# ml-unito/PartitionedLS.jl

Hardware: AMD Instinct MI355X
Metric: sign-pattern NNLS solves/sec (whole node); fp64 obj gap vs ref (higher is better)
Workload: dtype f64

## Files before the change

partitionedls.jl_amd/csrc/api.hip:

```cpp
#include "ctx.h"
#include <cstdarg>
#include <cstdio>
#include <cstdlib>
#include <cstring>
#include <new>

namespace partls {

static thread_local char g_err[512] = "";
static thread_local bool g_runtime_gone = false;
bool runtime_gone() { return g_runtime_gone; }
void set_error(const char *fmt, ...)
{
    va_list ap;
    va_start(ap, fmt);
    vsnprintf(g_err, sizeof(g_err), fmt, ap);
    va_end(ap);
}

void t_begin(partls_ctx *c, int w) { (void)hipEventRecord(c->ev0[w], c->stream); }
void t_end(partls_ctx *c, int w) { (void)hipEventRecord(c->ev1[w], c->stream); c->timed[w] = true; }
void t_collect(partls_ctx *c)
{
    for (int w = 0; w < PARTLS_T_COUNT; ++w)
        if (c->timed[w]) {
            float f = 0.f;
            if (hipEventElapsedTime(&f, c->ev0[w], c->ev1[w]) == hipSuccess) c->ms[w] = (double)f;
            c->timed[w] = false;
        }
}

partls_status check_common(partls_ctx *c, const void *X, int64_t N, int64_t M, int64_t ldX, const void *P, int64_t K, int64_t ldP)
{
    if (!c) { set_error("context is NULL"); return PARTLS_ERR_BAD_ARG; }
    if (!X || !P) { set_error("X or P is NULL"); return PARTLS_ERR_BAD_ARG; }
    if (N < 1 || M < 1 || K < 1) { set_error("need N, M, K >= 1 (got %lld, %lld, %lld)", (long long)N, (long long)M, (long long)K); return PARTLS_ERR_BAD_ARG; }
    if (ldX < N || ldP < M) { set_error("leading dimension smaller than the row count"); return PARTLS_ERR_BAD_ARG; }
    if (ldX >= ((int64_t)1 << 30)) { set_error("ldX = %lld: this build supports leading dimensions below 2^30 rows", (long long)ldX); return PARTLS_ERR_UNSUPPORTED; }
    if (K > 61) { set_error("K = %lld groups: this build supports K <= 61 (Alt, BnB, predict) and K <= 39 for the enumeration of fit(Opt)", (long long)K); return PARTLS_ERR_UNSUPPORTED; }
    if (M + 1 > 1023) { set_error("M = %lld features: this build supports M <= 1022", (long long)M); return PARTLS_ERR_UNSUPPORTED; }
    return PARTLS_OK;
}

double h_reg(const partls_ctx *c, int a, int b)
{
    double v = c->hG[(size_t)a * c->ldg + b];
    if (c->eta != 0.0 && a <= c->M && b <= c->M) v += c->eta * (double)__builtin_popcountll(c->mask_aug[a] & c->mask_aug[b]);
    return v;
}

}

using namespace partls;

extern "C" {

int partls_version(void) { return 105; }
const char *partls_last_error(void) { return g_err; }

int partls_device_count(void)
{
    int n = 0;
    if (hipGetDeviceCount(&n) != hipSuccess) return 0;
    return n;
}

partls_status partls_create(int device, partls_ctx **out)
try {
    if (!out) { set_error("partls_create: out is NULL"); return PARTLS_ERR_BAD_ARG; }
    *out = nullptr;
    int n = partls_device_count();
    if (n <= 0 || device < 0 || device >= n) {
        set_error("partls_create: no usable HIP device (count=%d, requested=%d); this library has no CPU fallback", n, device);
        return PARTLS_ERR_NO_DEVICE;
    }
    PARTLS_HIP_CHECK(hipSetDevice(device));
    partls_ctx *c = new (std::nothrow) partls_ctx();
    if (!c) { set_error("out of host memory"); return PARTLS_ERR_BAD_ARG; }
    c->device = device;
    if (hipDeviceGetAttribute(&c->ncu, hipDeviceAttributeMultiprocessorCount, device) != hipSuccess || c->ncu < 1) c->ncu = 256;
    if (const char *e = getenv("PARTLS_TOL_REL")) c->knobs.tol_rel = atof(e);
    if (const char *e = getenv("PARTLS_CHAIN_LEN")) c->knobs.chain_len = atoll(e);
    if (const char *e = getenv("PARTLS_GRID")) c->knobs.grid = atoll(e);
    if (const char *e = getenv("PARTLS_GRAM_S")) c->knobs.gram_S = atoi(e);
    if (const char *e = getenv("PARTLS_GRAM_CR")) c->knobs.gram_cr = atoi(e);
    if (const char *e = getenv("PARTLS_COOP_ROWS")) c->knobs.coop_rows = atoi(e);
    if (const char *e = getenv("PARTLS_PAIR")) c->knobs.pair = atoi(e) != 0 ? 1 : 0;
    if (const char *e = getenv("PARTLS_BIT_ORDER")) c->knobs.bit_order = !strcmp(e, "identity") ? 1 : (!strcmp(e, "calibrate") ? 2 : 0);
    if (const char *e = getenv("PARTLS_ALT_MS_MAX_ROUNDS")) c->knobs.alt_ms_max_rounds = atoi(e);
    if (const char *e = getenv("PARTLS_ALT_MS_CHUNK")) c->knobs.alt_ms_chunk = atoll(e);
    if (const char *e = getenv("PARTLS_KKT_TOL")) c->knobs.kkt_tol = atof(e);
    if (const char *e = getenv("PARTLS_NEAR_TIE_REL")) c->knobs.near_tie_rel = atof(e);
    if (const char *e = getenv("PARTLS_CAL_WB")) c->knobs.cal_wb = atof(e);
    if (const char *e = getenv("PARTLS_CAL_WS")) c->knobs.cal_ws = atof(e);
    c->knobs.no_coop = getenv("PARTLS_NO_COOP") != nullptr;
    c->knobs.no_export = getenv("PARTLS_NO_EXPORT") != nullptr;
    c->knobs.no_staged_upload = getenv("PARTLS_NO_STAGED_UPLOAD") != nullptr;
    if (const char *e = getenv("PARTLS_REG_MAXT")) { const int v = atoi(e); if (v >= 1 && v <= 20) c->knobs.reg_maxt = v; }
    c->knobs.eager_generic = getenv("PARTLS_EAGER_GENERIC") != nullptr;
    c->knobs.bnb_cold = getenv("PARTLS_BNB_COLD") != nullptr;
    if (const char *e = getenv("PARTLS_BNB_BATCH")) c->knobs.bnb_batch = atoi(e);
    if (const char *e = getenv("PARTLS_BNB_POOL_MB")) c->knobs.bnb_pool_mb = atoi(e);
    if (const char *e = getenv("PARTLS_BNB_WG_PER_CU")) c->knobs.bnb_wg_per_cu = atoi(e);
    if (const char *e = getenv("PARTLS_COOP_FAULT")) c->knobs.coop_fault = atoi(e);
    c->knobs.lz_fault = getenv("PARTLS_LZ_FAULT") != nullptr;
    c->knobs.no_tab_refine = getenv("PARTLS_NO_TAB_REFINE") != nullptr;
    c->knobs.finish_trace = getenv("PARTLS_FINISH_TRACE") != nullptr;
    c->knobs.alt_trace = getenv("PARTLS_ALT_TRACE") != nullptr;
    c->knobs.alt_always_check = getenv("PARTLS_ALT_ALWAYS_CHECK") != nullptr;
    c->knobs.print_stamps = getenv("PARTLS_PRINT_STAMPS") != nullptr;
    c->knobs.cv_serial = getenv("PARTLS_CV_SERIAL") != nullptr && strcmp(getenv("PARTLS_CV_SERIAL"), "0") != 0;
    c->knobs.resample_serial = getenv("PARTLS_RESAMPLE_SERIAL") != nullptr && strcmp(getenv("PARTLS_RESAMPLE_SERIAL"), "0") != 0;
    hipError_t e = hipStreamCreateWithFlags(&c->stream, hipStreamNonBlocking);
    for (int w = 0; w < PARTLS_T_COUNT && e == hipSuccess; ++w) {
        e = hipEventCreate(&c->ev0[w]);
        if (e == hipSuccess) e = hipEventCreate(&c->ev1[w]);
    }
    if (e != hipSuccess) {
        set_error("partls_create: stream / event creation failed: %s", hipGetErrorString(e));
        partls_destroy(c);
        return PARTLS_ERR_HIP;
    }
    *out = c;
    return PARTLS_OK;
}
PARTLS_ABI_GUARD

void partls_destroy(partls_ctx *c)
{
    if (!c) return;
    partls_destroy(c->cv_work);
    for (partls_ctx *v : c->cv_view) partls_destroy(v);
    c->cv_work = nullptr;
    c->cv_view.clear();
    int ndev = 0;
    const bool alive = hipGetDeviceCount(&ndev) == hipSuccess && ndev > c->device && hipSetDevice(c->device) == hipSuccess;
    if (alive && c->stream) (void)hipStreamSynchronize(c->stream);
    const hipStream_t stream = c->stream;
    hipEvent_t ev[2 * PARTLS_T_COUNT];
    for (int w = 0; w < PARTLS_T_COUNT; ++w) { ev[2 * w] = c->ev0[w]; ev[2 * w + 1] = c->ev1[w]; }
    g_runtime_gone = !alive;
    delete c;
    g_runtime_gone = false;
    if (alive) {
        for (hipEvent_t e : ev) if (e) (void)hipEventDestroy(e);
        if (stream) (void)hipStreamDestroy(stream);
    }
}

static partls_status predict_common(partls_ctx *c, const void *X, int64_t N, int64_t M, int64_t ldX, int x_on_device,
                                    const int64_t *P, int64_t K, int64_t ldP, const double *alpha, const double *beta, double t,
                                    double *yhat, bool x_f32 = false)
{
    partls_status st = check_common(c, X, N, M, ldX, P, K, ldP);
    if (st != PARTLS_OK) return st;
    if (!alpha || !beta || !yhat) { set_error("partls_predict: NULL argument"); return PARTLS_ERR_BAD_ARG; }
    PARTLS_HIP_CHECK(hipSetDevice(c->device));
    std::vector<double> w((size_t)M, 0.0);
    for (int64_t m = 0; m < M; ++m) {
        double s = 0.0;
        for (int64_t k = 0; k < K; ++k) {
            const int64_t v = P[m + k * ldP];
            if (v != 0 && v != 1) { set_error("P has an entry outside {0,1}"); return PARTLS_ERR_BAD_PARTITION; }
            s += (double)v * alpha[m] * beta[k];
        }
        w[(size_t)m] = s;
    }
    PARTLS_HIP_CHECK(c->wdev.ensure((size_t)(M + 1) * sizeof(double)));
    PARTLS_HIP_CHECK(hipMemcpyAsync(c->wdev.p, w.data(), (size_t)M * sizeof(double), hipMemcpyHostToDevice, c->stream));
    const void *dX = X;
    int64_t ld = ldX;
    double *dyh = yhat;
    if (!x_on_device) {
        const size_t esz = x_f32 ? sizeof(float) : sizeof(double);
        PARTLS_HIP_CHECK(c->predX.ensure((size_t)N * M * esz));
        PARTLS_HIP_CHECK(c->predY.ensure((size_t)N * sizeof(double)));
        const partls_status us = upload_matrix(c, c->predX.p, X, N, M, ldX, esz);
        if (us != PARTLS_OK) return us;
        dX = c->predX.p; ld = N; dyh = c->predY.as<double>();
    }
    PARTLS_HIP_CHECK(launch_residual(dX, N, M, ld, nullptr, c->wdev.as<double>(), t, nullptr, 1024, dyh, c->stream, nullptr, x_f32));
    if (!x_on_device)
        PARTLS_HIP_CHECK(hipMemcpyAsync(yhat, c->predY.p, (size_t)N * sizeof(double), hipMemcpyDeviceToHost, c->stream));
    PARTLS_HIP_CHECK(hipStreamSynchronize(c->stream));
    if (!x_on_device) { c->predX.release(); c->predY.release(); }
    return PARTLS_OK;
}

partls_status partls_predict(partls_ctx *c, const double *X, int64_t N, int64_t M, int64_t ldX, const int64_t *P, int64_t K,
                             int64_t ldP, const double *alpha, const double *beta, double t, double *yhat)
try {
    return predict_common(c, X, N, M, ldX, 0, P, K, ldP, alpha, beta, t, yhat);
}
PARTLS_ABI_GUARD

partls_status partls_predict_device(partls_ctx *c, const double *dX, int64_t N, int64_t M, int64_t ldX, const int64_t *P,
                                    int64_t K, int64_t ldP, const double *alpha, const double *beta, double t, double *dyhat)
try {
    return predict_common(c, dX, N, M, ldX, 1, P, K, ldP, alpha, beta, t, dyhat);
}
PARTLS_ABI_GUARD

partls_status partls_predict_f32(partls_ctx *c, const float *X, int64_t N, int64_t M, int64_t ldX, const int64_t *P, int64_t K,
                                 int64_t ldP, const double *alpha, const double *beta, double t, double *yhat)
try {
    return predict_common(c, X, N, M, ldX, 0, P, K, ldP, alpha, beta, t, yhat, true);
}
PARTLS_ABI_GUARD

partls_status partls_predict_device_f32(partls_ctx *c, const float *dX, int64_t N, int64_t M, int64_t ldX, const int64_t *P,
                                        int64_t K, int64_t ldP, const double *alpha, const double *beta, double t, double *dyhat)
try {
    return predict_common(c, dX, N, M, ldX, 1, P, K, ldP, alpha, beta, t, dyhat, true);
}
PARTLS_ABI_GUARD

partls_status partls_synth_truth(uint64_t seed, int64_t D, int64_t K, int64_t *P, double *wstar)
try {
    if (D < 1 || K < 1 || K > D) { set_error("partls_synth_truth: bad D/K"); return PARTLS_ERR_BAD_ARG; }
    std::vector<int64_t> grp((size_t)D);
    int64_t j = 0;
    for (int64_t k = 0; k < K; ++k) {
        const int64_t sz = D / K + ((k < D % K) ? 1 : 0);
        for (int64_t q = 0; q < sz; ++q) grp[(size_t)j++] = k;
    }
    if (P) {
        memset(P, 0, (size_t)D * K * sizeof(int64_t));
        for (int64_t m = 0; m < D; ++m) P[m + grp[(size_t)m] * D] = 1;
    }
    auto uni = [&](uint64_t stream, uint64_t idx) { return (double)(rnd64(seed, stream, idx) >> 11) * 0x1.0p-53; };
    if (wstar)
        for (int64_t k = 0; k < K; ++k) {
            double sum = 0.0;
            for (int64_t m = 0; m < D; ++m) if (grp[(size_t)m] == k) sum += uni(2, (uint64_t)m);
            const double bk = (uni(3, (uint64_t)k) - 0.5) * 10.0;
            for (int64_t m = 0; m < D; ++m) if (grp[(size_t)m] == k) wstar[m] = (uni(2, (uint64_t)m) / sum) * bk;
        }
    return PARTLS_OK;
}
PARTLS_ABI_GUARD

partls_status partls_synth_device(partls_ctx *c, uint64_t seed, int64_t N, int64_t D, const double *wstar, double *dX, double *dy)
try {
    if (!c || !wstar || !dX || !dy || N < 1 || D < 1) { set_error("partls_synth_device: bad argument"); return PARTLS_ERR_BAD_ARG; }
    PARTLS_HIP_CHECK(hipSetDevice(c->device));
    PARTLS_HIP_CHECK(c->wdev.ensure((size_t)D * sizeof(double)));
    PARTLS_HIP_CHECK(hipMemcpyAsync(c->wdev.p, wstar, (size_t)D * sizeof(double), hipMemcpyHostToDevice, c->stream));
    PARTLS_HIP_CHECK(launch_synth(seed, N, D, c->wdev.as<double>(), dX, dy, c->stream));
    PARTLS_HIP_CHECK(hipStreamSynchronize(c->stream));
    return PARTLS_OK;
}
PARTLS_ABI_GUARD

partls_status partls_get_timing(const partls_ctx *c, partls_timer which, double *ms)
try {
    if (!c || !ms || (int)which < 0 || (int)which >= PARTLS_T_COUNT) { set_error("partls_get_timing: bad argument"); return PARTLS_ERR_BAD_ARG; }
    *ms = c->ms[(int)which];
    return PARTLS_OK;
}
PARTLS_ABI_GUARD

partls_status partls_get_upload(const partls_ctx *c, double *ms, double *bytes)
try {
    if (!c || !ms || !bytes) { set_error("partls_get_upload: bad argument"); return PARTLS_ERR_BAD_ARG; }
    *ms = c->last_upload_ms; *bytes = c->last_upload_bytes;
    return PARTLS_OK;
}
PARTLS_ABI_GUARD

partls_status partls_get_pivots(const partls_ctx *c, int64_t *pivots)
try {
    if (!c || !pivots) { set_error("partls_get_pivots: bad argument"); return PARTLS_ERR_BAD_ARG; }
    *pivots = (int64_t)c->last_pivots;
    return PARTLS_OK;
}
PARTLS_ABI_GUARD

partls_status partls_get_kkt_violation(const partls_ctx *c, double *violation, double *min_pivot)
try {
    if (!c || !violation) { set_error("partls_get_kkt_violation: bad argument"); return PARTLS_ERR_BAD_ARG; }
    *violation = c->last_kkt;
    if (min_pivot) *min_pivot = c->last_min_loo;
    return PARTLS_OK;
}
PARTLS_ABI_GUARD

partls_status partls_get_vetoes(const partls_ctx *c, int64_t *vetoes)
try {
    if (!c || !vetoes) { set_error("partls_get_vetoes: bad argument"); return PARTLS_ERR_BAD_ARG; }
    *vetoes = (int64_t)c->last_vetoes;
    return PARTLS_OK;
}
PARTLS_ABI_GUARD

partls_status partls_get_blocks(const partls_ctx *c, int64_t *blocks)
try {
    if (!c || !blocks) { set_error("partls_get_blocks: bad argument"); return PARTLS_ERR_BAD_ARG; }
    *blocks = (int64_t)c->last_blocks;
    return PARTLS_OK;
}
PARTLS_ABI_GUARD

partls_status partls_get_sweep_route(const partls_ctx *c, int *kernel, int *tiles)
try {
    if (!c || !kernel || !tiles) { set_error("partls_get_sweep_route: bad argument"); return PARTLS_ERR_BAD_ARG; }
    const partls_ctx *p = c->prepared ? c : (c->cv_work && c->cv_work->prepared ? c->cv_work : nullptr);
    if (!p) { set_error("partls_get_sweep_route: context not prepared"); return PARTLS_ERR_STATE; }
    *kernel = p->use_reg ? (sweep_reg_small(p->T) ? PARTLS_ROUTE_REG_256 : PARTLS_ROUTE_REG_512)
                         : (p->knobs.eager_generic ? PARTLS_ROUTE_EAGER : PARTLS_ROUTE_DEFERRED);
    *tiles = p->use_reg ? p->T : 0;
    return PARTLS_OK;
}
PARTLS_ABI_GUARD

partls_status partls_get_near_ties(const partls_ctx *c, int64_t *evaluated)
try {
    if (!c || !evaluated) { set_error("partls_get_near_ties: bad argument"); return PARTLS_ERR_BAD_ARG; }
    *evaluated = c->last_near_evaluated;
    return PARTLS_OK;
}
PARTLS_ABI_GUARD

partls_status partls_get_gram(const partls_ctx *c, double *G_aug)
try {
    if (!c || !c->prepared || !G_aug) { set_error("partls_get_gram: context not prepared"); return PARTLS_ERR_STATE; }
    const int na = (int)c->M + 2;
    for (int j = 0; j < na; ++j)
        for (int i = 0; i < na; ++i) G_aug[(size_t)i + (size_t)j * na] = h_reg(c, i, j);
    return PARTLS_OK;
}
PARTLS_ABI_GUARD

}
```

partitionedls.jl_amd/csrc/common.h:

```cpp
#pragma once
#include <hip/hip_runtime.h>
#include <stdint.h>
#include <new>
#include <vector>
#include <string>
#include "../../include/partls.h"

namespace partls {

void set_error(const char *fmt, ...);
#define PARTLS_HIP_CHECK(expr)                                                                      \
    do {                                                                                            \
        hipError_t _e = (expr);                                                                     \
        if (_e != hipSuccess) {                                                                     \
            ::partls::set_error("%s failed: %s (%s:%d)", #expr, hipGetErrorString(_e), __FILE__, __LINE__); \
            return PARTLS_ERR_HIP;                                                                  \
        }                                                                                           \
    } while (0)
#define PARTLS_ABI_GUARD                                                                                                          \
    catch (const std::bad_alloc &) { ::partls::set_error("out of host memory"); return PARTLS_ERR_BAD_ARG; }                      \
    catch (...) { ::partls::set_error("internal error: an exception reached the C ABI"); return PARTLS_ERR_BAD_ARG; }

struct BitOrder { uint8_t gbit[40]; };

struct SweepParams {
    int n;
    int kbits;
    const uint64_t *mask;
    const double *T0;
    double *scratch;
    int64_t g_begin, g_end;
    int64_t chain_len;
    double tol;
    double piv_eps;
    int max_rounds;
    int pair;
    double *all_opt;
    double *best_obj;
    int64_t *best_pat;
    double *best_sol;
    double *second_obj;
    int64_t *second_pat;
    BitOrder rbit;
    unsigned long long *n_unconverged;
    unsigned long long *n_pivots;
    unsigned long long *n_vetoes;
    const int8_t *node_code;
    double *node_sol;
    double *node_obj2;
    int node_ld;
    double *node_tab;
    int8_t *node_basic;
    unsigned *node_piv;
    const double *const *node_src;
    double *const *node_dst;
    int resume;
    unsigned *grid_ctr;
    int coop_fault;
    int64_t batch_t0, batch_out;
    const double *batch_tol;
};

__device__ __forceinline__ bool ref_index_less(unsigned long long a, unsigned long long b, const unsigned char *rbit)
{
    unsigned long long d = a ^ b;
    int top = -1, at = 0;
    while (d) {
        const int i = __builtin_ctzll(d);
        d &= d - 1;
        const int r = rbit[i];
        if (r > top) { top = r; at = i; }
    }
    return top >= 0 && !((a >> at) & 1ULL);
}

hipError_t launch_sweep_generic(const SweepParams &p, int grid, hipStream_t s, bool models = false);
hipError_t launch_sweep_lazy(const SweepParams &p, int grid, hipStream_t s, bool models = false);
hipError_t launch_sweep_blk(const SweepParams &p, int T, int grid, hipStream_t s, bool models = false);
hipError_t launch_sweep_blk_batch(const SweepParams &p, int T, int grid, int batch, hipStream_t s);
hipError_t launch_layout_reg_batch(const double *Tfull, int n, int T, int batch, double *T0reg, hipStream_t s);
hipError_t launch_sweep_coop(const SweepParams &p, int nwg, hipStream_t s);
bool       sweep_reg_supported(int n);
int        sweep_reg_tiles(int n);
bool       sweep_reg_exports(int T);
bool       sweep_reg_small(int T);
size_t     sweep_reg_t0_doubles(int T);
int        sweep_reg_concurrency(int T);
hipError_t launch_layout_reg(const double *Tfull, int n, int T, double *T0reg, hipStream_t s);

size_t     gram_slab_doubles(int64_t N, int64_t M, int gram_S, int gram_cr, int *chunks_out, int *ldg_out);
hipError_t launch_gram(const void *X, int64_t N, int64_t M, int64_t ldX, const double *y, double *slab, int chunks,
                       int ldg, int gram_S, int gram_cr, double *G, hipStream_t s, const double *sw = nullptr, bool x_f32 = false);
hipError_t launch_gram_weightings(const double *X, int64_t N, int64_t M, int64_t ldX, const double *y, double *slab, int64_t slab_stride,
                                  int chunks, int ldg, int gram_S, int gram_cr, double *G, int64_t gstride, const double *sw, int batch,
                                  hipStream_t s);
int        weight_prep_blocks(int64_t N);
hipError_t launch_weightings_prep(const double *W, int64_t N, int64_t ldW, int batch, double *S, double *part, hipStream_t st);
inline hipError_t launch_weight_prep(const double *w, int64_t N, double *s, double *part, hipStream_t st) { return launch_weightings_prep(w, N, N, 1, s, part, st); }
hipError_t launch_oob_sse(const double *X, int64_t N, int64_t M, int64_t ldX, const double *y, const double *W, int64_t ldW,
                          const double *wv, int batch, double *part, hipStream_t st);

hipError_t launch_prep(const double *G, int ldg, int M, double eta, const uint64_t *mask_aug, int free_intercept,
                       const int *perm, double *scale, double *Tfull, int n, hipStream_t s);
hipError_t launch_prep_batch(const double *G, int64_t gstride, int E, int64_t q0, const double *eta, int ldg, int M, const uint64_t *mask_aug,
                             int free_intercept, const int *perm, double tol_rel, double *scale, double *Tfull, double *tol, int n,
                             int batch, hipStream_t s);

int        walk_flipped_bit(int chain, int step, int kbits, int seg_len, int nseg);
hipError_t launch_walk_codes(const uint64_t *mask, int n, int kbits, int chains, int L, int seg_len, int nseg, int8_t *codes, hipStream_t s);
hipError_t launch_pattern_gather(const double *in, int64_t npat, int kbits, const BitOrder &order, double *out, hipStream_t s);

hipError_t launch_models_cleanup(double *sol, const double *obj, int64_t g0, int64_t cnt, int M, int K, int kbits, const BitOrder &order,
                                 bool order_identity, const int *perm, const double *scale, const uint64_t *mask_aug, bool want_raw,
                                 double *out, hipStream_t s);

hipError_t launch_bnb_codes(const uint64_t *mask_tab, int n, const uint64_t *pat, const uint64_t *free_, int cnt, int8_t *codes, hipStream_t s);
hipError_t launch_bnb_nu(const double *sol, const double *obj2, int n, const double *scale, const uint64_t *mask_tab, int Kp,
                         const uint64_t *free_, int cnt, double *lb, int *branch, hipStream_t s);

hipError_t launch_gersh(const double *Tfull, int n, double *out, hipStream_t s);
hipError_t launch_alt_beta_system(const double *G, int ldg, int M, double eta, const uint64_t *mask_aug, const double *a, int Kp,
                                  double *GA, double *Hg, hipStream_t s);
hipError_t launch_alt_beta_system_batch(const double *G, int ldg, int M, double eta, const uint64_t *mask_aug, const double *a, int Kp,
                                        const int *slot, int cnt, double *GA, double *Hg, hipStream_t s);
hipError_t launch_alt_beta_system_problems(const double *G, int64_t gstride, int E, int64_t q0, const double *eta, const int *prob, int ldg,
                                           int M, const uint64_t *mask_aug, const double *a, int Kp, const int *slot, int cnt, double *GA,
                                           double *Hg, hipStream_t s);
hipError_t launch_residual(const void *X, int64_t N, int64_t M, int64_t ldX, const double *y, const double *w, double t,
                           double *partial, int nblocks, double *yhat, hipStream_t s, const double *wt = nullptr, bool x_f32 = false);
int        xtr_slices(int64_t N);
hipError_t launch_xtr(const void *X, int64_t N, int64_t M, int64_t ldX, const double *y, const double *yhat, double *gpart,
                      hipStream_t s, const double *wt = nullptr, bool x_f32 = false);
hipError_t launch_synth(uint64_t seed, int64_t N, int64_t D, const double *wstar_dev, double *X, double *y, hipStream_t s);

uint64_t rnd64(uint64_t seed, uint64_t stream, uint64_t idx);

}
```

partitionedls.jl_amd/csrc/ctx.h:

```cpp
#pragma once
#include "common.h"
#include <functional>
#include <vector>

namespace partls {

bool runtime_gone();
struct NoCopy {
    NoCopy() = default;
    NoCopy(const NoCopy &) = delete;
    NoCopy &operator=(const NoCopy &) = delete;
};

struct DevBuf : NoCopy {
    void *p = nullptr;
    size_t bytes = 0;
    ~DevBuf() { release(); }
    hipError_t ensure(size_t b)
    {
        if (b <= bytes && p) return hipSuccess;
        if (p) { hipError_t e = hipFree(p); p = nullptr; bytes = 0; if (e != hipSuccess) return e; }
        hipError_t e = hipMalloc(&p, b ? b : 8);
        if (e == hipSuccess) bytes = b;
        return e;
    }
    void release() { if (p && !runtime_gone()) (void)hipFree(p); p = nullptr; bytes = 0; }
    template <class T> T *as() const { return static_cast<T *>(p); }
};

struct DevChunks : NoCopy {
    std::vector<void *> v;
    ~DevChunks() { release(); }
    void release() { if (!runtime_gone()) for (void *q : v) (void)hipFree(q); v.clear(); }
    size_t size() const { return v.size(); }
    void push_back(void *q) { v.push_back(q); }
    void *operator[](size_t i) const { return v[i]; }
};

struct PinnedDoubles : NoCopy {
    double *p = nullptr;
    size_t cap = 0, n = 0, cap_prev = 0;
    ~PinnedDoubles() { release(); }
    hipError_t resize(size_t count)
    {
        if (count > cap) {
            if (p) (void)hipHostFree(p);
            p = nullptr; cap = 0;
            size_t want = count > 512 ? count : 512;
            if (want < 2 * cap_prev) want = 2 * cap_prev;
            hipError_t e = hipHostMalloc((void **)&p, want * sizeof(double), hipHostMallocDefault);
            if (e != hipSuccess) return e;
            cap = cap_prev = want;
        }
        n = count;
        return hipSuccess;
    }
    void release() { if (p && !runtime_gone()) (void)hipHostFree(p); p = nullptr; cap = n = 0; }
    double *data() const { return p; }
    size_t size() const { return n; }
    double &operator[](size_t i) const { return p[i]; }
};

template <class T> struct PinnedArray : NoCopy {
    T *p = nullptr;
    ~PinnedArray() { release(); }
    hipError_t alloc(size_t count)
    {
        release();
        const hipError_t e = hipHostMalloc((void **)&p, count * sizeof(T), hipHostMallocDefault);
        if (e != hipSuccess) p = nullptr;
        return e;
    }
    void release() { if (p && !runtime_gone()) (void)hipHostFree(p); p = nullptr; }
    operator T *() const { return p; }
};

struct UploadStaging : NoCopy {
    char *pin[8] = {};
    hipStream_t stream[4] = {};
    hipEvent_t event[8] = {};
    ~UploadStaging()
    {
        if (runtime_gone()) return;
        for (int i = 0; i < 8; ++i) { if (pin[i]) (void)hipHostFree(pin[i]); if (event[i]) (void)hipEventDestroy(event[i]); }
        for (int t = 0; t < 4; ++t) if (stream[t]) (void)hipStreamDestroy(stream[t]);
    }
};

}

struct partls_knobs {
    double tol_rel = 1e-11;
    long long chain_len = 0;
    long long grid = 0;
    int gram_S = 0, gram_cr = 0;
    int coop_rows = 0;
    bool no_coop = false;
    int reg_maxt = 18;
    bool no_staged_upload = false;
    bool no_export = false;
    bool eager_generic = false;
    int bnb_batch = 1024;
    int bnb_pool_mb = 65536;
    int bnb_wg_per_cu = 8;
    bool bnb_cold = false;
    bool lz_fault = false;
    int coop_fault = 0;
    bool no_tab_refine = false;
    bool finish_trace = false;
    bool alt_trace = false;
    bool alt_always_check = false;
    bool print_stamps = false;
    int alt_ms_max_rounds = 0;
    long long alt_ms_chunk = 0;
    double kkt_tol = 1e-12;
    double near_tie_rel = 1e-13;
    double cal_wb = 1.0, cal_ws = 1.0;
    bool cv_serial = false;
    bool resample_serial = false;
    int pair = -1;
    int bit_order = 0;
};

struct partls_ctx {
    int device = 0;
    int ncu = 256;
    partls_knobs knobs;
    hipStream_t stream = nullptr;
    hipEvent_t ev0[PARTLS_T_COUNT] = {}, ev1[PARTLS_T_COUNT] = {};
    bool timed[PARTLS_T_COUNT] = {};
    double ms[PARTLS_T_COUNT] = {};

    bool prepared = false;
    int64_t N = 0, M = 0, K = 0, ldX = 0;
    double eta = 0.0;
    uint32_t flags = 0;
    bool faithful = false;
    const void *dX = nullptr;
    bool x_f32 = false;
    const double *dy = nullptr;
    partls::DevBuf ownX, ownY;
    const double *dw = nullptr, *ds = nullptr;
    partls::DevBuf ownW, ownS, wPart;
    bool multi_rank = false;
    std::vector<int64_t> P;
    std::vector<uint64_t> mask_aug;
    std::vector<uint64_t> pack;
    const uint64_t *maskTabP = nullptr;
    const int *permP = nullptr;
    int ldg = 0, chunks = 0;
    partls::DevBuf slab, G, maskAugD , scale, Tfull, T0reg, scratch, bestObj, bestSol , bestPat, counters, allOpt,
        wdev, partial, yhatD, gD, nodeCode, nodeSol, nodeObj, predX, predY, gridCtr, nodeTab, nodeBasic, altA, altGA, altHg,
        nodePiv, maskInt, allOptRef, bnbIn, bnbOut, altGersh, amsState, amsWork;
    partls::DevChunks bnbChunks;
    size_t bnbSlotBytes = 0, bnbMaxSlots = 0;
    int bnbChunkSlots = 512;
    std::vector<int> bnbFree, bnbRefs;
    std::vector<partls_ctx *> peers;
    partls::PinnedDoubles hPart, hGpart;
    partls::PinnedDoubles sweepOut, nodeOut, exportSol;
    partls::DevBuf mdlRows, mdlOut, mdlCtr;
    partls::PinnedDoubles mdlStage;
    std::function<partls_status(partls_ctx *)> gram_hook;
    partls::PinnedDoubles amsHostIn, amsHostOut;
    partls::PinnedDoubles bnbHostIn, bnbHostOut;
    partls::UploadStaging up;
    double last_upload_ms = 0.0, last_upload_bytes = 0.0;
    partls::PinnedDoubles hG;
    partls::PinnedDoubles hScale;
    int n = 0, kbits = 0, T = 0;
    std::vector<int> perm;
    std::vector<uint64_t> mask_tab;
    bool use_reg = false;
    partls::BitOrder order{};
    bool order_ready = false, order_identity = true;
    std::vector<double> flip_cost;
    double tol = 0.0;
    unsigned long long last_pivots = 0, last_vetoes = 0, last_blocks = 0;
    std::vector<int64_t> near_pat;
    int64_t near_for = -1;
    std::vector<std::pair<double, int64_t>> cand;
    int64_t last_near_evaluated = 0;
    int export_wg = -1;
    double last_kkt = 0.0;
    double last_min_loo = 0.0;
    unsigned long long sweep_vetoes = 0;
    bool coop_state_valid = false;
    bool coop_fallback = false;
    partls::PinnedArray<double> hTab;
    partls::PinnedArray<int8_t> hBasic;
    size_t hTabDoubles = 0;
    bool tab_valid = false, tab_full = false;
    partls_ctx *cv_work = nullptr;
    std::vector<partls_ctx *> cv_view;
    partls::DevBuf cvG, cvBatch, cvEta;
    partls::PinnedDoubles cvHost, cvHostG;
    partls::DevBuf rsW, rsS, rsPart, rsWv;
    partls::PinnedDoubles rsHost;
};

namespace partls {

void t_begin(partls_ctx *c, int w);
void t_end(partls_ctx *c, int w);
void t_collect(partls_ctx *c);

partls_status ctx_prepare(partls_ctx *c, const void *X, int64_t N, int64_t M, int64_t ldX, const double *y, int x_on_device,
                          const int64_t *P, int64_t K, int64_t ldP, double eta, bool faithful, uint32_t flags, const double *w = nullptr,
                          bool x_f32 = false);
void forget_problem(partls_ctx *c);
partls_status adopt_or_upload(partls_ctx *c, const void *X, int64_t N, int64_t M, int64_t ldX, const double *y, int x_on_device, size_t esz);
partls_status prepare_weights(partls_ctx *c, const double *w, int64_t N, int on_device);
partls_status ctx_prepare_tableau(partls_ctx *c);
partls_status load_partition(partls_ctx *c, const int64_t *P, int64_t M, int64_t K, int64_t ldP);
partls_status upload_matrix(partls_ctx *c, void *dst, const void *X, int64_t N, int64_t M, int64_t ldX, size_t esz = sizeof(double));
constexpr double SWEEP_PIV_EPS = 1e-11;
inline int sweep_max_rounds(int n) { return 20 * (n + 1); }
SweepParams sweep_params(const partls_ctx *c, bool internal_order);
partls_status ensure_sweep_scratch(partls_ctx *c, int grid);
partls_status node_sweep_params(partls_ctx *c, size_t nodes, int64_t chain_len, int grid, SweepParams *p);
inline void bind_counters(SweepParams &p, unsigned long long *w) { p.n_unconverged = w; p.n_pivots = w + 1; p.n_vetoes = w + 2; }
struct SweepBlock { unsigned long long *counters; double *best_obj; int64_t *best_pat; double *second_obj; int64_t *second_pat; };
inline size_t sweep_block_words(int grid, bool runner_up) { return 4 + (runner_up ? 4 : 2) * (size_t)grid; }
inline SweepBlock sweep_block(double *base, int grid, bool runner_up)
{
    double *b = base + 4;
    const size_t g = (size_t)grid;
    return {reinterpret_cast<unsigned long long *>(base), b, reinterpret_cast<int64_t *>(b + g), runner_up ? b + 2 * g : nullptr,
            runner_up ? reinterpret_cast<int64_t *>(b + 3 * g) : nullptr};
}
void bind_sweep_block(SweepParams &p, double *base, int grid, bool runner_up);
hipError_t launch_any_sweep(partls_ctx *c, SweepParams &p, int grid, bool models = false);
partls_status calibrate_bit_order(partls_ctx *c);
bool sweep_plan(partls_ctx *c, int64_t total, int64_t *chain_len_out, int *grid_out, const char *who);
bool sweep_pairs(const partls_ctx *c, int64_t total);
int64_t reference_pattern(const partls_ctx *c, int64_t q);
void install_sweep_result(partls_ctx *c, const double *sweep_out, int grid, bool has_sol, double *bobj_out, int64_t *bpat_out);

struct CvOut {
    std::vector<double> alpha, beta, t, opt, sse;
    std::vector<int64_t> best;
    std::vector<int32_t> status;
    void assign(int64_t B, int64_t M, int64_t K);
    void deliver(int64_t B, int64_t M, int64_t K, double *alpha_out, int64_t ld_alpha, double *beta_out, int64_t ld_beta, double *t_out,
                 double *opt_out, int64_t *best_out, double *sse_out, int32_t *status_out) const;
};
struct ProblemBatch {
    int64_t B = 0, E = 1;
    const double *eta = nullptr;
    const double *G = nullptr, *hostG = nullptr;
    int64_t gs = 0;
    bool serial = false;
    const char *who = "";
    std::function<partls_status(int64_t q, int64_t bpat, int64_t unconv)> finish;
};
partls_status make_internal(partls_ctx *c, partls_ctx **slot);
partls_status cv_check_inputs(const char *who, partls_ctx *c, const double *X, int64_t N, int64_t M, int64_t ldX, const double *y,
                              const int64_t *P, int64_t K, int64_t ldP, const int64_t *fold_ptr, int64_t F, const double *eta, int64_t E);
partls_status cv_grams(partls_ctx *c, const double *X, int64_t N, int64_t M, int64_t ldX, const double *y, const double *w, int x_on_device,
                       int64_t K, const int64_t *fold_ptr, int64_t F, uint32_t flags, const char *who, int *ldg_out, int *chunks_out);
void cv_point_rows(partls_ctx *c, partls_ctx *W, const int64_t *fold_ptr, int64_t F, int64_t f);
void batch_reset(partls_ctx *c, int64_t N, int64_t M, int64_t K, uint32_t flags);
partls_status batch_calibrate(partls_ctx *c, const int64_t *P, int64_t ldP, uint32_t flags, int ldg, int chunks, const ProblemBatch &pb,
                              int64_t cal_gram, const std::function<void(partls_ctx *)> &point_rows);
partls_status batch_sweep(partls_ctx *c, const ProblemBatch &pb);
partls_status finish_model(partls_ctx *c, int64_t q, int64_t bpat, int64_t unconv, CvOut &o);
void model_weights(const partls_ctx *work, const CvOut &o, int64_t q, double *w);

partls_status solve_nodes(partls_ctx *c, const std::vector<int8_t> &codes, size_t cnt, std::vector<double> &sols,
                          std::vector<double> &obj2, unsigned long long *unconv, bool resume = false, bool want_tab = false);
partls_status solve_nodes_device(partls_ctx *c, size_t cnt, const int8_t *code, double *obj2, double *sol,
                                 unsigned long long *counters, int max_rounds);
partls_status solve_nodes_device_at(partls_ctx *c, const double *T0reg, double tol, size_t cnt, const int8_t *code, double *obj2,
                                    double *sol, unsigned long long *counters, int max_rounds);

struct AltProblems {
    int64_t B = 1, E = 1, q0 = 0;
    const double *G = nullptr;
    int64_t gs = 0;
    const double *eta = nullptr;
    const double *scale = nullptr;
    const double *T0reg = nullptr;
    size_t t0d = 0;
    const double *tol = nullptr;
    const double *yy = nullptr;
};
struct AltTables {
    double *alpha_all; int64_t ld_alpha_all; double *beta_all; int64_t ld_beta_all;
    double *t_all, *opt_all; int64_t *iters_all; int32_t *status_all;
};
struct AltWinner {
    int64_t start = -1, iters = 0;
    double opt = 0.0;
    std::vector<double> a, b, wv, hdiag;
    std::vector<int8_t> vcode;
};
partls_status alt_multistart_core(partls_ctx *c, const AltProblems *pp, double eps, int64_t T, int64_t R,
                                  const double *alpha0, int64_t ld_alpha0, const double *beta0, int64_t ld_beta0,
                                  const AltTables &tb, AltWinner *win);
partls_status alt_finish(partls_ctx *c, const std::vector<double> &a, const std::vector<double> &b, const std::vector<double> &wv,
                         const std::vector<int8_t> &vcode_last, const std::vector<double> &hdiag, const std::vector<double> &gersh,
                         double optval, int64_t iters_done, unsigned long long unconv_total,
                         double *alpha, double *beta, double *t, double *opt, int64_t *iters);
void opt_codes(const partls_ctx *c, uint64_t pattern, std::vector<int8_t> &codes);

void unscale_solution(const partls_ctx *c, const double *sol, std::vector<double> &w);
partls_status data_pass(partls_ctx *c, const std::vector<double> &w, bool want_obj, bool want_grad, double *obj2, std::vector<double> *g,
                        const std::function<void()> &overlap);
partls_status data_objective(partls_ctx *c, const std::vector<double> &w, double *opt, std::vector<double> *grad = nullptr);
bool kkt_says_ill_conditioned(const partls_ctx *c);
double kkt_violation_data(const partls_ctx *c, const std::vector<double> &w, const std::vector<double> &g, const std::vector<int8_t> &code,
                          int *worst);
struct RefineOut { bool have = false; double obj = 0.0; std::vector<double> g; };
partls_status refine_solution(partls_ctx *c, std::vector<double> &w, bool free_intercept, int steps = 2, RefineOut *out = nullptr);
double h_reg(const partls_ctx *c, int a, int b);
partls_status check_common(partls_ctx *c, const void *X, int64_t N, int64_t M, int64_t ldX, const void *P, int64_t K, int64_t ldP);

}
```

partitionedls.jl_amd/csrc/opt.hip:

```cpp
#include "ctx.h"
#include "near_tie.h"
#include "sweep_rules.h"
#include <algorithm>
#include <chrono>
#include <cmath>
#include <cstdio>
#include <cstring>
#include <functional>
#include <thread>

namespace partls {

static bool opt_range_ok(const partls_ctx *c, const char *who)
{
    if (c->kbits <= 40) return true;
    set_error("%s: %d sign bits: the enumeration of 2^(K+1) patterns is out of range (K <= 39); fit(Alt) and fit(BnB) take up to 61 groups", who, c->kbits);
    return false;
}

static void cleanup_opt(const partls_ctx *c, const std::vector<double> &w, uint64_t pattern, double *alpha, double *beta, double *t)
{
    const int64_t M = c->M, K = c->K;
    std::vector<double> a((size_t)M, 0.0);
    for (int64_t m = 0; m < M; ++m) {
        const int f = sign_of_var(c->mask_aug[(size_t)m], pattern);
        a[(size_t)m] = (f != 0) ? w[(size_t)m] / (double)f : 0.0;
        if (a[(size_t)m] < 0.0) a[(size_t)m] = 0.0;
    }
    std::vector<double> A((size_t)K, 0.0);
    for (int64_t k = 0; k < K; ++k) {
        double s = 0.0;
        for (int64_t m = 0; m < M; ++m) s += (double)c->P[(size_t)m + (size_t)k * M] * a[(size_t)m];
        const double sk = ((pattern >> k) & 1ULL) ? 1.0 : -1.0;
        beta[k] = sk * s;
        A[(size_t)k] = (s == 0.0) ? 1.0 : s;
    }
    for (int64_t m = 0; m < M; ++m) {
        double s = 0.0;
        for (int64_t k = 0; k < K; ++k) s += (double)c->P[(size_t)m + (size_t)k * M] * a[(size_t)m] / A[(size_t)k];
        alpha[m] = s;
    }
    *t = w[(size_t)M];
}

}

using namespace partls;

extern "C" {

partls_status partls_opt_prepare(partls_ctx *c, const double *X, int64_t N, int64_t M, int64_t ldX, const double *y,
                                 int x_on_device, const int64_t *P, int64_t K, int64_t ldP, double eta, uint32_t flags)
try {
    return ctx_prepare(c, X, N, M, ldX, y, x_on_device, P, K, ldP, eta, (flags & PARTLS_OPT_FAITHFUL_INTERCEPT) != 0, flags);
}
PARTLS_ABI_GUARD

partls_status partls_opt_prepare_weighted(partls_ctx *c, const double *X, int64_t N, int64_t M, int64_t ldX, const double *y,
                                          const double *w, int x_on_device, const int64_t *P, int64_t K, int64_t ldP, double eta,
                                          uint32_t flags)
try {
    return ctx_prepare(c, X, N, M, ldX, y, x_on_device, P, K, ldP, eta, (flags & PARTLS_OPT_FAITHFUL_INTERCEPT) != 0, flags, w);
}
PARTLS_ABI_GUARD

partls_status partls_opt_prepare_f32(partls_ctx *c, const float *X, int64_t N, int64_t M, int64_t ldX, const double *y, const double *w,
                                     int x_on_device, const int64_t *P, int64_t K, int64_t ldP, double eta, uint32_t flags)
try {
    return ctx_prepare(c, X, N, M, ldX, y, x_on_device, P, K, ldP, eta, (flags & PARTLS_OPT_FAITHFUL_INTERCEPT) != 0, flags, w, true);
}
PARTLS_ABI_GUARD

int64_t partls_opt_num_patterns(const partls_ctx *c) { return (c && c->prepared && c->kbits <= 40) ? ((int64_t)1 << c->kbits) : 0; }

partls_status partls_opt_sweep(partls_ctx *c, int64_t g_begin, int64_t g_end, double *best_obj, int64_t *best_pattern,
                               double *all_opt, int64_t *n_unconverged)
try {
    if (!c || !c->prepared) { set_error("partls_opt_sweep: context not prepared"); return PARTLS_ERR_STATE; }
    if (!opt_range_ok(c, "partls_opt_sweep")) return PARTLS_ERR_UNSUPPORTED;
    const int64_t npat = (int64_t)1 << c->kbits;
    if (g_end < 0) g_end = npat;
    if (g_begin < 0 || g_begin > g_end || g_end > npat) { set_error("bad Gray-index range [%lld,%lld)", (long long)g_begin, (long long)g_end); return PARTLS_ERR_BAD_ARG; }
    if (all_opt && !c->faithful) { set_error("all_opt needs PARTLS_OPT_FAITHFUL_INTERCEPT"); return PARTLS_ERR_BAD_ARG; }
    PARTLS_HIP_CHECK(hipSetDevice(c->device));
    if (g_begin == g_end) {
        if (best_obj) *best_obj = INFINITY;
        if (best_pattern) *best_pattern = -1;
        if (n_unconverged) *n_unconverged = 0;
        return PARTLS_OK;
    }
    if (!c->order_ready) {
        partls_status st = calibrate_bit_order(c);
        if (st != PARTLS_OK) return st;
    }
    const int n = c->n;
    const int64_t total = g_end - g_begin;
    int64_t chain_len = 0;
    int grid = 0;
    if (!sweep_plan(c, total, &chain_len, &grid, "partls_opt_sweep")) return PARTLS_ERR_UNSUPPORTED;

    const size_t sweep_words = sweep_block_words(grid, true);
    PARTLS_HIP_CHECK(c->bestObj.ensure(sizeof(double) * sweep_block_words(std::max(grid, 4096), true)));
    PARTLS_HIP_CHECK(hipMemsetAsync(c->bestObj.p, 0, 4 * sizeof(unsigned long long), c->stream));
    if (all_opt) {
        PARTLS_HIP_CHECK(c->allOpt.ensure((size_t)npat * sizeof(double)));
        if (total < npat) PARTLS_HIP_CHECK(hipMemsetAsync(c->allOpt.p, 0xFF, (size_t)npat * sizeof(double), c->stream));
    }
    const partls_status ss = ensure_sweep_scratch(c, grid);
    if (ss != PARTLS_OK) return ss;

    SweepParams p = sweep_params(c, true);
    p.g_begin = g_begin; p.g_end = g_end; p.chain_len = chain_len;
    p.pair = sweep_pairs(c, total) ? 1 : 0;
    p.all_opt = all_opt ? c->allOpt.as<double>() : nullptr;
    bind_sweep_block(p, c->bestObj.as<double>(), grid, true);
    if (!c->use_reg && c->knobs.lz_fault) p.coop_fault = 77;
    c->export_wg = -1;
    if (((c->use_reg && (sweep_reg_small(c->T) || sweep_reg_exports(c->T))) || (!c->use_reg && !c->knobs.eager_generic)) && !c->knobs.no_export) {
        PARTLS_HIP_CHECK(c->bestSol.ensure((size_t)grid * n * sizeof(double)));
        p.best_sol = c->bestSol.as<double>();
        p.node_ld = n;
    }

    t_begin(c, PARTLS_T_SWEEP);
    PARTLS_HIP_CHECK(launch_any_sweep(c, p, grid));
    t_end(c, PARTLS_T_SWEEP);

    unsigned long long cnt[3] = {0, 0, 0};
    PARTLS_HIP_CHECK(c->sweepOut.resize(sweep_words));
    const double *sweep_out = c->sweepOut.data();
    PARTLS_HIP_CHECK(hipMemcpyAsync(c->sweepOut.data(), c->bestObj.p, sweep_words * sizeof(double), hipMemcpyDeviceToHost, c->stream));
    if (all_opt) {
        const void *src = c->allOpt.p;
        if (!c->order_identity) {
            PARTLS_HIP_CHECK(c->allOptRef.ensure((size_t)npat * sizeof(double)));
            PARTLS_HIP_CHECK(launch_pattern_gather(c->allOpt.as<double>(), npat, c->kbits, c->order, c->allOptRef.as<double>(), c->stream));
            src = c->allOptRef.p;
        }
        PARTLS_HIP_CHECK(hipMemcpyAsync(all_opt, src, (size_t)npat * sizeof(double), hipMemcpyDeviceToHost, c->stream));
    }
    PARTLS_HIP_CHECK(hipStreamSynchronize(c->stream));
    t_collect(c);
    std::memcpy(cnt, sweep_out, sizeof(cnt));
    if (c->knobs.print_stamps) {
        double st[32] = {0};
        if (hipMemcpy(st, c->scratch.p, sizeof(st), hipMemcpyDeviceToHost) == hipSuccess)
            fprintf(stderr, "[partls stamps] scan: pre %.0f barrier %.0f post %.0f | gather: work %.0f barrier %.0f | panel: work %.0f barrier %.0f | "
                            "update %.0f | scatter %.0f | chain-load %.0f/%.0f | pivots %llu || gather split: block setup %.0f chain %.0f rhs/myj %.0f"
                            " || workgroup 0: %.0f blocks, %.0f scans, %.0f pivots || pair walk: twin scan %.0f, solve + rows + scan %.0f\n",
                    st[9], st[10], st[0], st[12] + st[13] + st[8], st[1], st[11], st[2], st[3], st[4], st[5], st[6], cnt[1], st[12], st[13], st[8],
                    st[24], st[25], st[26], st[15], st[14]);
    }
    double bobj = INFINITY;
    int64_t bpat = -1;
    install_sweep_result(c, sweep_out, grid, p.best_sol != nullptr, &bobj, &bpat);
    if (best_obj) *best_obj = bobj;
    if (best_pattern) *best_pattern = bpat;
    if (n_unconverged) *n_unconverged = (int64_t)cnt[0];
    return PARTLS_OK;
}
PARTLS_ABI_GUARD

partls_status partls_opt_finish(partls_ctx *c, int64_t pattern, double *alpha, double *beta, double *t, double *opt,
                                int64_t *best_index)
try {
    if (!c || !c->prepared) { set_error("partls_opt_finish: context not prepared"); return PARTLS_ERR_STATE; }
    if (!alpha || !beta || !t || !opt) { set_error("partls_opt_finish: NULL output"); return PARTLS_ERR_BAD_ARG; }
    if (pattern < 0 || pattern >= ((int64_t)1 << (c->K + 1))) { set_error("pattern out of range"); return PARTLS_ERR_BAD_ARG; }
    PARTLS_HIP_CHECK(hipSetDevice(c->device));
    const uint64_t kmask = ((uint64_t)1 << c->kbits) - 1;
    uint64_t used = 1ULL << c->K;
    for (int i = 0; i < c->n; ++i) if (c->hScale[(size_t)i] != 0.0) used |= c->mask_tab[(size_t)i];

    std::vector<uint64_t> cands{(uint64_t)pattern & kmask & used};
    if (pattern == c->near_for)
        for (int64_t q : c->near_pat) {
            const uint64_t v = (uint64_t)q & kmask & used;
            if (std::find(cands.begin(), cands.end(), v) == cands.end()) cands.push_back(v);
        }
    const int export_wg = (pattern == c->near_for) ? c->export_wg : -1;
    c->export_wg = -1;
    c->near_for = -1;
    c->near_pat.clear();
    c->last_near_evaluated = (int64_t)cands.size();

    t_begin(c, PARTLS_T_FINISH);
    const auto f0 = std::chrono::steady_clock::now();
    std::vector<double> sols, obj2, w, wbest, g, gbest;
    std::vector<int8_t> codes;
    unsigned long long unconv = 0, unconv_best = 0;
    double obest = INFINITY, loo_best = 0.0;
    uint64_t pbest = cands[0];
    for (size_t ci = 0; ci < cands.size(); ++ci) {
        partls_status st = PARTLS_OK;
        bool taken = false;
        if (ci == 0 && export_wg >= 0) {
            PARTLS_HIP_CHECK(c->exportSol.resize((size_t)c->n));
            PARTLS_HIP_CHECK(hipMemcpyAsync(c->exportSol.data(), c->bestSol.as<double>() + (size_t)export_wg * c->n, (size_t)c->n * sizeof(double), hipMemcpyDeviceToHost, c->stream));
            PARTLS_HIP_CHECK(hipStreamSynchronize(c->stream));
            sols.assign(c->exportSol.data(), c->exportSol.data() + c->n);
            opt_codes(c, cands[ci], codes);
            taken = true;
            double smax = 0.0;
            for (int i = 0; i < c->n; ++i) smax = std::max(smax, std::fabs(sols[(size_t)i]));
            for (int i = 0; i < c->n && taken; ++i) {
                const double v = sols[(size_t)i];
                if (!std::isfinite(v)) taken = false;
                else if (v != 0.0 && (codes[(size_t)i] == 0 || (codes[(size_t)i] == 1 && v < -1e-9 * smax) || (codes[(size_t)i] == -1 && v > 1e-9 * smax))) taken = false;
            }
            if (taken) { c->tab_valid = false; unconv = 0; }
            if (c->knobs.finish_trace) fprintf(stderr, "[finish] the sweep's solution of its winner (workgroup %d): %s\n", export_wg, taken ? "taken" : "refused (signs), solving again");
        }
        if (!taken) {
            opt_codes(c, cands[ci], codes);
            st = solve_nodes(c, codes, 1, sols, obj2, &unconv, false, true);
            if (st != PARTLS_OK) return st;
        }
        unscale_solution(c, sols.data(), w);
        RefineOut ro;
        st = refine_solution(c, w, !c->faithful, 2, &ro);
        if (st != PARTLS_OK) return st;
        double o = 0.0;
        if (ro.have) { o = ro.obj; g.swap(ro.g); }
        else { st = data_objective(c, w, &o, &g); if (st != PARTLS_OK) return st; }
        if (c->knobs.finish_trace && cands.size() > 1) fprintf(stderr, "[finish] near tie: pattern %llu data objective %.17g\n", (unsigned long long)cands[ci], o);
        if (ci == 0 || o < obest || (o == obest && cands[ci] < pbest)) { obest = o; pbest = cands[ci]; wbest = w; gbest = g; unconv_best = unconv; loo_best = c->last_min_loo; }
    }
    const auto f1 = std::chrono::steady_clock::now();
    uint64_t full = pbest;
    if (!c->faithful) { if (wbest[(size_t)c->M] > 0.0) full |= (1ULL << c->K); }
    full &= used;
    std::vector<int8_t> vcode((size_t)c->M + 1, 0);
    for (int64_t m = 0; m <= c->M; ++m) {
        if (m == c->M && !c->faithful) { vcode[(size_t)m] = 2; continue; }
        const int f = sign_of_var(c->mask_aug[(size_t)m], full);
        vcode[(size_t)m] = (int8_t)((f > 0) - (f < 0));
    }
    int worst = -1;
    c->last_kkt = kkt_violation_data(c, wbest, gbest, vcode, &worst);
    *opt = obest;
    if (c->knobs.finish_trace) {
        const auto f2 = std::chrono::steady_clock::now();
        auto ms = [](auto a, auto b) { return std::chrono::duration<double, std::milli>(b - a).count(); };
        fprintf(stderr, "[finish] %zu candidate(s): solve + refine + data objective / gradient %.3f ms, KKT check %.3f ms; data-space KKT violation %.3e (variable %d)\n",
                cands.size(), ms(f0, f1), ms(f1, f2), c->last_kkt, worst);
    }
    t_end(c, PARTLS_T_FINISH);
    PARTLS_HIP_CHECK(hipStreamSynchronize(c->stream));
    t_collect(c);
    cleanup_opt(c, wbest, full, alpha, beta, t);
    if (best_index) *best_index = (int64_t)full;
    if (unconv_best) { set_error("winner re-solve hit the pivot cap"); return PARTLS_ERR_NOT_CONVERGED; }
    c->last_min_loo = loo_best;
    if (kkt_says_ill_conditioned(c)) {
        set_error("the winner's KKT conditions do not hold in data space (violation %.2e of ||x|| ||y|| at variable %d, tolerance %.1e; %llu columns "
                  "refused as dependent in the sweep): X is too ill-conditioned for the fp64 Gram form (cond(X) >~ 1e6); the outputs hold the best "
                  "Gram-form model", c->last_kkt, worst, c->knobs.kkt_tol, c->sweep_vetoes);
        return PARTLS_ERR_ILL_CONDITIONED;
    }
    return PARTLS_OK;
}
PARTLS_ABI_GUARD

partls_status partls_opt_pattern(partls_ctx *c, int64_t pattern, double *raw_alpha, double *optval)
try {
    if (!c || !c->prepared) { set_error("partls_opt_pattern: context not prepared"); return PARTLS_ERR_STATE; }
    if (!c->faithful) { set_error("partls_opt_pattern needs a context prepared with PARTLS_OPT_FAITHFUL_INTERCEPT"); return PARTLS_ERR_STATE; }
    if (pattern < 0 || pattern >= ((int64_t)1 << c->kbits)) { set_error("pattern out of range"); return PARTLS_ERR_BAD_ARG; }
    PARTLS_HIP_CHECK(hipSetDevice(c->device));
    std::vector<double> sols, obj2, w;
    unsigned long long unconv = 0;
    std::vector<int8_t> codes;
    opt_codes(c, (uint64_t)pattern, codes);
    partls_status st = solve_nodes(c, codes, 1, sols, obj2, &unconv, false, true);
    if (st != PARTLS_OK) return st;
    unscale_solution(c, sols.data(), w);
    st = refine_solution(c, w, false);
    if (st != PARTLS_OK) return st;
    if (optval) { st = data_objective(c, w, optval); if (st != PARTLS_OK) return st; }
    if (raw_alpha)
        for (int64_t m = 0; m <= c->M; ++m) {
            const int f = sign_of_var(c->mask_aug[(size_t)m], (uint64_t)pattern);
            const double a = (f != 0) ? w[(size_t)m] / (double)f : 0.0;
            raw_alpha[m] = a > 0.0 ? a : 0.0;
        }
    if (unconv) { set_error("pattern solve hit the pivot cap"); return PARTLS_ERR_NOT_CONVERGED; }
    return PARTLS_OK;
}
PARTLS_ABI_GUARD

static void par_rows(int64_t rows, size_t row_bytes, const std::function<void(int64_t, int64_t)> &fn)
{
    const int nt = (size_t)rows * row_bytes < ((size_t)32 << 20) ? 1 : 8;
    if (nt == 1) { fn(0, rows); return; }
    std::vector<std::thread> th;
    const int64_t per = (rows + nt - 1) / nt;
    try {
        for (int i = 1; i < nt; ++i) {
            const int64_t r0 = std::min<int64_t>(rows, i * per), r1 = std::min<int64_t>(rows, r0 + per);
            th.emplace_back(fn, r0, r1);
        }
    } catch (...) {
        const int64_t done_from = (int64_t)(th.size() + 1) * per;
        fn(std::min<int64_t>(rows, done_from), rows);
    }
    fn(0, std::min<int64_t>(rows, per));
    for (std::thread &t : th) t.join();
}

static void copy_rows(double *dst, int64_t ld_dst, const double *src, int64_t width, int64_t rows)
{
    if (!dst || width <= 0) return;
    par_rows(rows, (size_t)width * sizeof(double), [&](int64_t r0, int64_t r1) {
        if (ld_dst == width) std::memcpy(dst + (size_t)r0 * width, src + (size_t)r0 * width, (size_t)(r1 - r0) * width * sizeof(double));
        else for (int64_t r = r0; r < r1; ++r) std::memcpy(dst + (size_t)r * ld_dst, src + (size_t)r * width, (size_t)width * sizeof(double));
    });
}

partls_status partls_opt_models(partls_ctx *c, int64_t g_begin, int64_t g_end, int64_t *pattern, double *optval, double *raw_alpha,
                                int64_t ld_raw, double *alpha, int64_t ld_alpha, double *beta, int64_t ld_beta, double *t,
                                int64_t *n_unconverged, int64_t *n_vetoes)
try {
    if (!c || !c->prepared) { set_error("partls_opt_models: context not prepared"); return PARTLS_ERR_STATE; }
    if (!c->faithful) { set_error("partls_opt_models needs a context prepared with PARTLS_OPT_FAITHFUL_INTERCEPT"); return PARTLS_ERR_STATE; }
    if (!opt_range_ok(c, "partls_opt_models")) return PARTLS_ERR_UNSUPPORTED;
    const int64_t npat = (int64_t)1 << c->kbits, M = c->M, K = c->K;
    if (g_end < 0) g_end = npat;
    if (g_begin < 0 || g_begin > g_end || g_end > npat) { set_error("partls_opt_models: bad Gray-index range [%lld,%lld)", (long long)g_begin, (long long)g_end); return PARTLS_ERR_BAD_ARG; }
    if (!pattern) { set_error("partls_opt_models: pattern is NULL"); return PARTLS_ERR_BAD_ARG; }
    if ((alpha || beta || t) && !(alpha && beta && t)) { set_error("partls_opt_models: alpha, beta and t go together (all three or none)"); return PARTLS_ERR_BAD_ARG; }
    if ((raw_alpha && ld_raw < M + 1) || (alpha && (ld_alpha < M || ld_beta < K))) { set_error("partls_opt_models: leading dimension too small"); return PARTLS_ERR_BAD_ARG; }
    if (n_unconverged) *n_unconverged = 0;
    if (n_vetoes) *n_vetoes = 0;
    PARTLS_HIP_CHECK(hipSetDevice(c->device));
    if (g_begin == g_end) return PARTLS_OK;
    if (!c->order_ready) {
        partls_status st = calibrate_bit_order(c);
        if (st != PARTLS_OK) return st;
    }
    const int n = c->n;
    const int64_t total = g_end - g_begin;
    const size_t out_w = 3 + (size_t)M + (size_t)K;
    const size_t per_pat = (size_t)n + 1 + out_w;
    const int64_t cap = std::max<int64_t>(1, (int64_t)(PARTLS_OPT_MODELS_PIECE_BYTES / (per_pat * sizeof(double))));
    const int64_t npieces = (total + cap - 1) / cap;
    const int64_t piece = (total + npieces - 1) / npieces;
    PARTLS_HIP_CHECK(c->mdlRows.ensure((size_t)piece * (n + 1) * sizeof(double)));
    PARTLS_HIP_CHECK(c->mdlOut.ensure((size_t)piece * out_w * sizeof(double)));
    const size_t stage_words = 4 + (size_t)piece * (out_w + (raw_alpha ? (size_t)n : 0));
    PARTLS_HIP_CHECK(c->mdlStage.resize(stage_words));
    if (!c->use_reg) c->coop_state_valid = false;
    unsigned long long unconv = 0, vetoes = 0;
    for (int64_t p0 = g_begin; p0 < g_end; p0 += piece) {
        const int64_t cnt = std::min<int64_t>(piece, g_end - p0);
        int64_t chain_len = 0;
        int grid = 0;
        if (!sweep_plan(c, cnt, &chain_len, &grid, "partls_opt_models")) return PARTLS_ERR_UNSUPPORTED;
        PARTLS_HIP_CHECK(c->mdlCtr.ensure(sizeof(double) * sweep_block_words(grid, false)));
        PARTLS_HIP_CHECK(hipMemsetAsync(c->mdlCtr.p, 0, 4 * sizeof(unsigned long long), c->stream));
        const partls_status ss = ensure_sweep_scratch(c, grid);
        if (ss != PARTLS_OK) return ss;
        double *rows = c->mdlRows.as<double>(), *obj = rows + (size_t)cnt * n, *out = c->mdlOut.as<double>();
        SweepParams p = sweep_params(c, true);
        p.g_begin = p0; p.g_end = p0 + cnt; p.chain_len = chain_len;
        bind_sweep_block(p, c->mdlCtr.as<double>(), grid, false);
        p.node_sol = rows; p.node_obj2 = obj; p.node_ld = n;
        PARTLS_HIP_CHECK(launch_any_sweep(c, p, grid, true));
        PARTLS_HIP_CHECK(launch_models_cleanup(rows, obj, p0, cnt, (int)M, (int)K, c->kbits, c->order, c->order_identity, c->permP,
                                               c->scale.as<double>(), c->maskAugD.as<uint64_t>(), raw_alpha != nullptr, out, c->stream));
        double *st = c->mdlStage.data();
        PARTLS_HIP_CHECK(hipMemcpyAsync(st, c->mdlCtr.p, 4 * sizeof(double), hipMemcpyDeviceToHost, c->stream));
        PARTLS_HIP_CHECK(hipMemcpyAsync(st + 4, out, (size_t)cnt * out_w * sizeof(double), hipMemcpyDeviceToHost, c->stream));
        if (raw_alpha) PARTLS_HIP_CHECK(hipMemcpyAsync(st + 4 + (size_t)cnt * out_w, rows, (size_t)cnt * n * sizeof(double), hipMemcpyDeviceToHost, c->stream));
        PARTLS_HIP_CHECK(hipStreamSynchronize(c->stream));
        unsigned long long cn[3];
        std::memcpy(cn, st, sizeof(cn));
        unconv += cn[0];
        vetoes += cn[2];
        const double *o = st + 4;
        const size_t r = (size_t)(p0 - g_begin);
        std::memcpy(pattern + r, o, (size_t)cnt * sizeof(int64_t));
        if (optval) std::memcpy(optval + r, o + cnt, (size_t)cnt * sizeof(double));
        if (t) std::memcpy(t + r, o + 2 * cnt, (size_t)cnt * sizeof(double));
        if (alpha) {
            copy_rows(alpha + r * ld_alpha, ld_alpha, o + 3 * cnt, M, cnt);
            copy_rows(beta + r * ld_beta, ld_beta, o + 3 * cnt + (size_t)cnt * M, K, cnt);
        }
        if (raw_alpha) copy_rows(raw_alpha + r * ld_raw, ld_raw, o + (size_t)cnt * out_w, M + 1, cnt);
    }
    if (n_unconverged) *n_unconverged = (int64_t)unconv;
    if (n_vetoes) *n_vetoes = (int64_t)vetoes;
    return PARTLS_OK;
}
PARTLS_ABI_GUARD

partls_status partls_fit_opt(partls_ctx *c, const double *X, int64_t N, int64_t M, int64_t ldX, const double *y,
                             const int64_t *P, int64_t K, int64_t ldP, double eta, uint32_t flags,
                             double *alpha, double *beta, double *t, double *opt, int64_t *best_index, double *all_opt)
try {
    if (all_opt) flags |= PARTLS_OPT_FAITHFUL_INTERCEPT;
    partls_status st = partls_opt_prepare(c, X, N, M, ldX, y, 0, P, K, ldP, eta, flags);
    if (st != PARTLS_OK) return st;
    double bobj; int64_t bpat, unconv;
    st = partls_opt_sweep(c, 0, -1, &bobj, &bpat, all_opt, &unconv);
    if (st != PARTLS_OK) return st;
    if (bpat < 0) { set_error("sweep produced no candidate"); return PARTLS_ERR_NOT_CONVERGED; }
    st = partls_opt_finish(c, bpat, alpha, beta, t, opt, best_index);
    if (st != PARTLS_OK) return st;
    if (unconv) { set_error("%lld subproblems hit the pivot cap", (long long)unconv); return PARTLS_ERR_NOT_CONVERGED; }
    return PARTLS_OK;
}
PARTLS_ABI_GUARD

partls_status partls_opt_bit_order(partls_ctx *c, int64_t *gbit, double *flip_cost)
try {
    if (!c || !c->prepared) { set_error("partls_opt_bit_order: context not prepared"); return PARTLS_ERR_STATE; }
    if (!gbit) { set_error("partls_opt_bit_order: gbit is NULL"); return PARTLS_ERR_BAD_ARG; }
    if (!opt_range_ok(c, "partls_opt_bit_order")) return PARTLS_ERR_UNSUPPORTED;
    PARTLS_HIP_CHECK(hipSetDevice(c->device));
    if (!c->order_ready) {
        partls_status st = calibrate_bit_order(c);
        if (st != PARTLS_OK) return st;
    }
    for (int k = 0; k < c->kbits; ++k) {
        gbit[k] = c->order.gbit[k];
        if (flip_cost) flip_cost[k] = c->flip_cost.empty() ? -1.0 : c->flip_cost[(size_t)k];
    }
    return PARTLS_OK;
}
PARTLS_ABI_GUARD

partls_status partls_opt_candidates(const partls_ctx *c, int64_t capacity, double *obj, int64_t *pattern, int64_t *count)
try {
    if (!c || !c->prepared || !count || capacity < 0 || (capacity > 0 && (!obj || !pattern))) { set_error("partls_opt_candidates: bad argument"); return PARTLS_ERR_BAD_ARG; }
    const int64_t n = std::min<int64_t>(capacity, (int64_t)c->cand.size());
    for (int64_t i = 0; i < n; ++i) { obj[i] = c->cand[(size_t)i].first; pattern[i] = c->cand[(size_t)i].second; }
    *count = n;
    return PARTLS_OK;
}
PARTLS_ABI_GUARD

partls_status partls_opt_merge_candidates(partls_ctx *c, int64_t count, const double *obj, const int64_t *pattern, double *win_obj, int64_t *win_pattern)
try {
    if (!c || !c->prepared || count < 0 || (count > 0 && (!obj || !pattern))) { set_error("partls_opt_merge_candidates: bad argument"); return PARTLS_ERR_BAD_ARG; }
    std::vector<std::pair<double, int64_t>> all;
    for (int64_t i = 0; i < count; ++i) if (pattern[i] >= 0 && obj[i] == obj[i]) all.emplace_back(obj[i], pattern[i]);
    const int64_t local_winner = c->cand.empty() ? -1 : c->cand[0].second;
    c->near_pat.clear();
    c->cand.clear();
    if (all.empty()) { c->near_for = -1; c->export_wg = -1; if (win_obj) *win_obj = INFINITY; if (win_pattern) *win_pattern = -1; return PARTLS_OK; }
    const std::pair<double, int64_t> win = *std::min_element(all.begin(), all.end());
    const double bobj = win.first;
    const int64_t bpat = win.second;
    const double yy = h_reg(c, (int)c->M + 1, (int)c->M + 1);
    const double lim2 = bobj * bobj + c->knobs.near_tie_rel * (yy > 0.0 ? yy : 0.0);
    install_near_ties(win, std::move(all), lim2, 3, c->cand, c->near_pat, c->near_for);
    if (local_winner != bpat) c->export_wg = -1;
    if (win_obj) *win_obj = bobj;
    if (win_pattern) *win_pattern = bpat;
    return PARTLS_OK;
}
PARTLS_ABI_GUARD

}
```

partitionedls.jl_amd/csrc/sweep_blk.hip:

```cpp
#include "sweep_rules.h"
#include <atomic>
#include <type_traits>

namespace partls {
namespace blk {

static constexpr int THREADS = 512;
static constexpr int MAXT = 20;
#ifndef PARTLS_UPD_UNROLL
#define PARTLS_UPD_UNROLL 1
#endif
static constexpr int MB = 8;
#ifndef PARTLS_EXPORT_BIG
#define PARTLS_EXPORT_BIG 1
#endif
#ifndef PARTLS_MERGED_SCAN
#define PARTLS_MERGED_SCAN 1
#endif
#ifndef PARTLS_LANE_MASKS
#define PARTLS_LANE_MASKS 1
#endif
#ifndef PARTLS_MB_BIG
#define PARTLS_MB_BIG 8
#endif
#ifndef PARTLS_PAIR
#define PARTLS_PAIR 1
#endif
static constexpr int EXPORT_MAXT = 17;
static constexpr int MBB = PARTLS_MB_BIG;
static constexpr int NO_VETO = 99;
static constexpr int PAIR_MAXC = 16;
static constexpr int PAIR_PIV_MIN_HI = 0x3f1a36e2;
static constexpr int F64_EXP_HI = 0x7ff00000;

constexpr int nslots(int T) { return T * (T + 1) / 2; }
constexpr int tri(int g) { return g * (g + 1) / 2; }
constexpr int split(int T)
{
    int best = 1, bestmax = 1 << 30;
    for (int g = 1; g < T; ++g) {
        int a = tri(g), b = nslots(T) - tri(g);
        int m = a > b ? a : b;
        if (m < bestmax) { bestmax = m; best = g; }
    }
    return T == 1 ? 1 : best;
}
constexpr int rstride(int T) { return (T % 2) ? T : T + 1; }
constexpr int colw(int T) { return 513; }
static constexpr int MAXT_S = 10;
static constexpr int CW_S = 257;
template <class PT> __device__ __forceinline__ PT *uniform_ptr(PT *p)
{
    const unsigned long long v = (unsigned long long)p;
    const unsigned lo = (unsigned)__builtin_amdgcn_readfirstlane((int)v), hi = (unsigned)__builtin_amdgcn_readfirstlane((int)(v >> 32));
    return (PT *)(((unsigned long long)hi << 32) | lo);
}

#ifdef PARTLS_STAMPS
#define STAMP_DECL unsigned long long st_acc[24] = {0, 0, 0, 0, 0, 0, 0, 0, 0, 0, 0, 0, 0, 0, 0, 0, 0, 0, 0, 0, 0, 0, 0, 0}; unsigned long long st_t = __builtin_amdgcn_s_memtime();
#define STAMP(ph) do { __builtin_amdgcn_sched_barrier(0); unsigned long long _n = __builtin_amdgcn_s_memtime(); \
                       st_acc[ph] += _n - st_t; st_t = _n; __builtin_amdgcn_sched_barrier(0); } while (0)
#ifndef PARTLS_STAMP_TID
#define PARTLS_STAMP_TID 0
#endif
#define STAMP_FLUSH do { if (tid == PARTLS_STAMP_TID && blockIdx.x == 0 && p.scratch) { for (int _i = 0; _i < 24; ++_i) p.scratch[_i] = (double)st_acc[_i]; \
                                p.scratch[24] = (double)bc; p.scratch[25] = (double)sc; p.scratch[26] = (double)npiv; } } while (0)
#else
#define STAMP_DECL
#define STAMP(ph) do { } while (0)
#define STAMP_FLUSH do { } while (0)
#endif

static constexpr int CWMAX = colw(MAXT);
template <int CWX, int MAXTX>
struct LdsImageT {
    double Z[MB * CWX];
    double U[2 * (MB + 64)];
    double Dinv[MB + 64];
    unsigned long long s_inf[32];
    unsigned long long s_bas[16];
    unsigned long long s_sum[16];
    int s_veto[2];
    double s_best[4];
    unsigned char s_rbit[64];
    unsigned long long s_vmask[16 * MAXTX];
    double Pbase[2 * MB * CWX];
};
struct LdsImage {
    double Z[MBB * CWMAX];
    double U[2 * (MBB + 64)];
    double Dinv[MBB + 64];
    unsigned long long s_inf[32];
    unsigned long long s_bas[16];
    unsigned long long s_sum[16];
    int s_veto[2];
    double s_best[4];
    unsigned char s_rbit[64];
    unsigned long long s_vmask[16 * MAXT];
    double Pbase[2 * MBB * CWMAX];
};
static_assert(2 * MBB >= PAIR_MAXC, "the pair walk gathers up to PAIR_MAXC columns into the two panel buffers");
__shared__ LdsImage lds_image;
__shared__ LdsImageT<CW_S, MAXT_S> lds_small;

template <int W>
__device__ __forceinline__ auto *image_of()
{
    if constexpr (W == 1) return &lds_small; else return &lds_image;
}

template <int T, int H, int W = 2>
struct Half {
    static constexpr int G = W == 1 ? T : split(T);
    static constexpr int GLO = H ? G : 0;
    static constexpr int GHI = H ? T : G;
    static constexpr int OFF = H ? tri(G) : 0;
    static constexpr int CNT = (H ? nslots(T) - tri(G) : tri(G)) > 0 ? (H ? nslots(T) - tri(G) : tri(G)) : 1;
    static constexpr int XN = GHI;
    static constexpr int RS = rstride(T);
    static constexpr int CW = W == 1 ? CW_S : colw(T);
    static constexpr int NT = W == 1 ? 256 : THREADS;
    __device__ static constexpr int idx(int rho, int gam) { return tri(gam) + rho - OFF; }
};

template <class L>
__device__ __forceinline__ void tiles_store(double *dst, const double (&S)[L::CNT], int t8)
{
    double *bp = uniform_ptr(dst) + (size_t)L::OFF * 256;
#pragma unroll
    for (int s = 0; s < L::CNT; ++s) {
        if ((s & 1) == 0) asm volatile("" : "+s"(bp));
        bp[(s & 1) * 256 + t8] = S[s];
        if (s & 1) bp += 512;
    }
}

template <int T, int H, int W, int KAPPA, class SA>
__device__ __forceinline__ void gather_tile(const SA &S, double *P, int a, int b, unsigned pm)
{
    using L = Half<T, H, W>;
    if constexpr (KAPPA >= L::GLO && KAPPA < L::GHI) {
        if ((pm >> b) & 1u) {
            double *col = P + __builtin_popcount(pm & ((1u << b) - 1u)) * L::CW + a * L::RS;
#pragma unroll
            for (int rho = 0; rho <= KAPPA; ++rho) col[rho] = S[L::idx(rho, KAPPA)];
        }
    }
    if ((pm >> a) & 1u) {
        double *col = P + __builtin_popcount(pm & ((1u << a) - 1u)) * L::CW + b * L::RS;
#pragma unroll
        for (int gam = (KAPPA + 1 > L::GLO ? KAPPA + 1 : L::GLO); gam < L::GHI; ++gam) col[gam] = S[L::idx(KAPPA, gam)];
    }
}

template <int T, int H, int W, int KAPPA, class SA>
__device__ __forceinline__ void scatter_tile(SA &S, const double *P, int a, int b, unsigned pm)
{
    using L = Half<T, H, W>;
    if constexpr (KAPPA >= L::GLO && KAPPA < L::GHI) {
        if ((pm >> b) & 1u) {
            const double *col = P + __builtin_popcount(pm & ((1u << b) - 1u)) * L::CW + a * L::RS;
#pragma unroll
            for (int rho = 0; rho <= KAPPA; ++rho) S[L::idx(rho, KAPPA)] = col[rho];
        }
    }
    if ((pm >> a) & 1u) {
        const double *col = P + __builtin_popcount(pm & ((1u << a) - 1u)) * L::CW + b * L::RS;
#pragma unroll
        for (int gam = (KAPPA > L::GLO ? KAPPA : L::GLO); gam < L::GHI; ++gam) S[L::idx(KAPPA, gam)] = col[gam];
    }
}

template <int M, int CW, int MBK>
__device__ __forceinline__ int panel_block(double *P, double *Z, double *U, double *Dinv, int myj, bool my_basic,
                                           double piv_eps, int tid, int prow, bool idle_wave)
{
    if (idle_wave) {
#pragma unroll
        for (int s = 0; s < M; ++s) __syncthreads();
        return M;
    }
    constexpr int US = MBK + 64;
    const int dummy = MBK + (tid & 63);
    double pv[M];
#pragma unroll
    for (int j = 0; j < M; ++j) pv[j] = P[j * CW + prow];
    const int uslot = myj >= 0 ? myj : dummy;
    int veto = M;
#pragma unroll
    for (int s = 0; s < M; ++s) {
        Z[s * CW + prow] = pv[s];
        U[(s & 1) * US + uslot] = pv[s];
        if (myj == s) {
            const double d = pv[s];
            Dinv[s] = (my_basic || d > piv_eps) ? rcp_newton(d) : 0.0;
        }
        __syncthreads();
        double inv = Dinv[s];
        double u[M];
#pragma unroll
        for (int j = 0; j < M; ++j) u[j] = U[(s & 1) * US + j];
        asm volatile("" : "+v"(inv));
#pragma unroll
        for (int j = 0; j < M; ++j) asm volatile("" : "+v"(u[j]));
        if ((pv[s] * pv[s]) * (inv * piv_eps) >= 1.0) veto = veto < s ? veto : s;
        if (__builtin_amdgcn_readfirstlane(__double2hiint(inv)) & 0x7ff00000) {
            const double ainv = fabs(inv), fz = -pv[s] * inv;
            if (myj == s) {
#pragma unroll
                for (int j = 0; j < M; ++j) pv[j] = (j == s) ? -inv : u[j] * ainv;
            } else {
#pragma unroll
                for (int j = 0; j < M; ++j) pv[j] = (j == s) ? pv[s] * ainv : fma(fz, u[j], pv[j]);
            }
        }
    }
#pragma unroll
    for (int j = 0; j < M; ++j) P[j * CW + prow] = pv[j];
    return veto;
}

template <int CW>
__device__ __forceinline__ void pair_solve(const double *P, const int *cpos, int m, int lane, int rhspos, double *out)
{
    const int r = lane & 15, h = lane >> 4;
    const int code = cpos[r < m ? r : 0];
    const unsigned basm = (unsigned)__ballot(code < 0 && lane < m);
    const int pos = code < 0 ? ~code : code;
    double pv[4];
#pragma unroll
    for (int jj = 0; jj < 4; ++jj) {
        const int c = 4 * h + jj;
        const double v = P[c * CW + pos];
        pv[jj] = (r < m && c < m) ? v : 0.0;
    }
    double qc = P[r * CW + rhspos];
    if (r >= m) qc = 0.0;
    bool hard = false;
#pragma unroll 1
    for (int s = 0; s < m; ++s) {
        const double d = readlane_f64(pv[0], s);
        const int dh = __double2hiint(d);
        if ((!((basm >> s) & 1u) && !(dh > PAIR_PIV_MIN_HI)) || (dh & F64_EXP_HI) == F64_EXP_HI) { hard = true; break; }
        const double inv = rcp_newton(d), ainv = fabs(inv);
        const double pvs = __shfl(pv[0], r);
        const double fz = -pvs * inv;
        const double qs = readlane_f64(qc, s);
        double val[4];
#pragma unroll
        for (int jj = 0; jj < 4; ++jj) {
            const double u = __shfl(pv[0], (s + 4 * h + jj) & 15);
            val[jj] = (r == s) ? u * ainv : fma(fz, u, pv[jj]);
        }
        if (h == 0) val[0] = (r == s) ? -inv : pvs * ainv;
        qc = (r == s) ? qs * ainv : fma(fz, qs, qc);
        const double nx = __shfl(val[0], (lane + 16) & 63);
        pv[0] = val[1]; pv[1] = val[2]; pv[2] = val[3]; pv[3] = nx;
    }
    if (lane < PAIR_MAXC) {
        out[PAIR_MAXC + lane] = qc;
        out[lane] = ((basm >> lane) & 1u) ? -qc : qc;
    }
    if (lane == 0) out[2 * PAIR_MAXC + 1] = hard ? 1.0 : 0.0;
}

#define PARTLS_CASES(M) M(0) M(1) M(2) M(3) M(4) M(5) M(6) M(7) M(8) M(9) M(10) M(11) M(12) M(13) M(14) M(15) M(16) M(17) M(18) M(19)

template <int T, int H, bool NODE, int W = 2, bool MODELS = false, bool BATCH = false, bool PAIRK = false>
__device__ __forceinline__ void sweep_body(const SweepParams &p)
{
    using L = Half<T, H, W>;
    constexpr int RS = L::RS, CW = L::CW, RHSPOS = 16 * RS, NW = (T + 3) / 4;
    constexpr int THREADS = L::NT;
    constexpr int MB = W == 1 ? blk::MB : MBB;
    static_assert(!(NODE && MODELS), "node mode exports no per-pattern models (finish_pattern's capped flag is chain mode's)");
    constexpr bool MERGED = PARTLS_MERGED_SCAN && !NODE && !BATCH && T <= 17;
    constexpr bool LANE_MASKS = PARTLS_LANE_MASKS && !BATCH && T <= 16;
    constexpr bool PAIR = PAIRK && PARTLS_PAIR && MERGED && LANE_MASKS && W == 2 && !MODELS;
    static_assert(PAIR == PAIRK, "the pair walk is launched only where it is compiled (pair_compiled)");
    static_assert(W == 2 || RHSPOS < 256, "the 256-thread kernel needs every panel row position (and the rhs row) below 256");
    auto &lds_image = *image_of<W>();
    const int tid = threadIdx.x, t8 = tid & 255, a = t8 & 15, b = t8 >> 4, lane = tid & 63, wave = tid >> 6;
    const int n = p.n;
    const int nwords = (n + 63) >> 6;

    double *const Pbase = lds_image.Pbase, *const Z = lds_image.Z, *const U = lds_image.U, *const Dinv = lds_image.Dinv;
    unsigned long long *const s_inf = lds_image.s_inf, *const s_bas = lds_image.s_bas, *const s_vmask = lds_image.s_vmask;
    unsigned long long *const s_sum = lds_image.s_sum;
    int *const s_veto = lds_image.s_veto;
    double *const s_best = lds_image.s_best;
    [[maybe_unused]] double *const s_pair = U;
    [[maybe_unused]] int *const s_cpos = reinterpret_cast<int *>(Dinv);
    [[maybe_unused]] int *const s_tw = s_cpos + PAIR_MAXC;
    static_assert(2 * (MB + 64) >= 2 * PAIR_MAXC + 2, "pair_solve's `out` (doubles) fits U");
    static_assert(2 * (MB + 64) >= PAIR_MAXC + 8, "s_cpos and s_tw (PAIR_MAXC + 8 ints) fit Dinv (MB + 64 doubles)");
    for (int i = tid; i < 2 * MB * CW; i += THREADS) Pbase[i] = 0.0;
    for (int i = tid; i < MB * CW; i += THREADS) Z[i] = 0.0;
    if (tid < 2 * (MB + 64)) U[tid] = 0.0;
    if (tid < MB + 64) Dinv[tid] = 0.0;
    if (tid < 32) s_inf[tid] = 0;
    if (tid < 16) { s_bas[tid] = 0; s_sum[tid] = 0; }
    if (tid < 2) s_veto[tid] = NO_VETO;
    if (tid == 0) {
        s_best[0] = __builtin_inf(); reinterpret_cast<long long *>(s_best)[1] = -1;
        s_best[2] = __builtin_inf(); reinterpret_cast<long long *>(s_best)[3] = -1;
    }
    if (tid < 16 * T) s_vmask[tid] = tid < p.n ? p.mask[tid] : 0ULL;
    if (tid < 64) lds_image.s_rbit[tid] = tid < 40 ? p.rbit.gbit[tid] : 0;
    __syncthreads();

    double S[L::CNT];
    double q = 0.0, corner = 0.0;
    double mybest = __builtin_inf();
    const bool has_var = tid < n;
    bool basic = false, blocked = false;
    const int mypos = (tid & 15) * RS + (tid >> 4);
    const int rowc = tid / RS, rowrho = tid - rowc * RS;
    const bool idle_wave = __builtin_amdgcn_readfirstlane((tid & ~63) > RHSPOS ? 1 : 0) != 0;

    unsigned npiv = 0, nunconv = 0, nveto = 0;
    unsigned bc = 0, sc = 0;

    const int clen = (int)p.chain_len;
    const int nchains = (int)((p.g_end - p.g_begin + clen - 1) / clen);

    STAMP_DECL
    for (int chain = blockIdx.x; chain < nchains; chain += gridDim.x) {
        const int64_t g0 = p.g_begin + (int64_t)chain * clen;
        const int glen = (int)((g0 + clen < p.g_end) ? clen : p.g_end - g0);
        STAMP(5);
        const double *src = p.T0;
        if constexpr (NODE) {
            if (p.node_src) {
                const double *snap = p.node_src[chain];
                if (snap) src = snap;
            }
        }
        {
            const double *bp = uniform_ptr(src) + (size_t)L::OFF * 256;
#pragma unroll
            for (int s = 0; s < L::CNT; ++s) {
                if ((s & 1) == 0) asm volatile("" : "+s"(bp));
                S[s] = bp[(s & 1) * 256 + t8];
                if (s & 1) bp += 512;
            }
        }
        q = (tid < 16 * T) ? src[(size_t)nslots(T) * 256 + tid] : 0.0;
        corner = src[(size_t)nslots(T) * 256 + 16 * T];
        basic = false;
        if constexpr (NODE) {
            if (src != p.T0 && tid < 16 * T) basic = reinterpret_cast<const int8_t *>(src + (nslots(T) * 256 + 16 * T + 8))[tid] != 0;
        }
        STAMP(6);

        auto finish_pattern = [&](int gi, [[maybe_unused]] bool capped) {
            const uint64_t g = (uint64_t)g0 + (unsigned)gi;
            const uint64_t pat = NODE ? (uint64_t)chain : g ^ (g >> 1);
            const double obj2 = corner > 0.0 ? corner : 0.0;
            if constexpr (NODE) {
                if (p.node_piv && tid == 0) {
                    unsigned *o = p.node_piv + 3 * ((size_t)chain * clen + gi);
                    o[0] = npiv; o[1] = bc; o[2] = sc;
                }
            }
            if (p.all_opt && tid == THREADS - 1) p.all_opt[pat] = sqrt(obj2);
            if constexpr (MODELS) {
                const size_t row = (size_t)chain * (size_t)clen + (size_t)gi;
                if (has_var) p.node_sol[row * p.node_ld + tid] = capped ? __builtin_nan("") : (basic ? q : 0.0);
                if (tid == THREADS - 1) p.node_obj2[row] = capped ? __builtin_nan("") : sqrt(obj2);
            }
            if constexpr (!NODE && !MODELS && (W == 1 || (PARTLS_EXPORT_BIG && T <= EXPORT_MAXT))) {
                if (p.best_sol && obj2 < mybest) {
                    mybest = obj2;
                    if (has_var) p.best_sol[(size_t)blockIdx.x * p.node_ld + tid] = basic ? q : 0.0;
                }
            }
            if (tid == THREADS - 1 && obj2 <= s_best[2]) {
                const double bo = s_best[0];
                const long long bp = reinterpret_cast<long long *>(s_best)[1];
                if (obj2 < bo || (obj2 == bo && ref_index_less(pat, (unsigned long long)bp, lds_image.s_rbit))) {
                    s_best[2] = bo; reinterpret_cast<long long *>(s_best)[3] = bp;
                    s_best[0] = obj2; reinterpret_cast<long long *>(s_best)[1] = (long long)pat;
                } else if (obj2 < s_best[2] || ref_index_less(pat, (unsigned long long)reinterpret_cast<long long *>(s_best)[3], lds_image.s_rbit)) {
                    s_best[2] = obj2; reinterpret_cast<long long *>(s_best)[3] = (long long)pat;
                }
            }
        };
        [[maybe_unused]] auto record_twin = [&](int gi, double cornerv, double qv, bool bv) {
            const uint64_t g = (uint64_t)g0 + (unsigned)gi;
            const uint64_t pat = g ^ (g >> 1);
            const double obj2 = cornerv > 0.0 ? cornerv : 0.0;
            if (p.all_opt && tid == THREADS - 1) p.all_opt[pat] = sqrt(obj2);
            if constexpr (PARTLS_EXPORT_BIG && T <= EXPORT_MAXT) {
                if (p.best_sol && obj2 < mybest) {
                    mybest = obj2;
                    if (has_var) p.best_sol[(size_t)blockIdx.x * p.node_ld + tid] = bv ? qv : 0.0;
                }
            }
            if (tid == THREADS - 1 && obj2 <= s_best[2]) {
                const double bo = s_best[0];
                const long long bp = reinterpret_cast<long long *>(s_best)[1];
                if (obj2 < bo || (obj2 == bo && ref_index_less(pat, (unsigned long long)bp, lds_image.s_rbit))) {
                    s_best[2] = bo; reinterpret_cast<long long *>(s_best)[3] = bp;
                    s_best[0] = obj2; reinterpret_cast<long long *>(s_best)[1] = (long long)pat;
                } else if (obj2 < s_best[2] || ref_index_less(pat, (unsigned long long)reinterpret_cast<long long *>(s_best)[3], lds_image.s_rbit)) {
                    s_best[2] = obj2; reinterpret_cast<long long *>(s_best)[3] = (long long)pat;
                }
            }
        };
        int gi = 0;
        [[maybe_unused]] bool tw_pending = false;
        [[maybe_unused]] int pr_ncol = -1;
        [[maybe_unused]] auto pair_partner = [&](int i) -> int {
            const int j = (((unsigned)g0 + (unsigned)i) & 1u) ? i - 1 : i + 1;
            return (PAIR && j >= 0 && j < glen) ? j : -1;
        };
        [[maybe_unused]] auto pair_unit_end = [&](int i) -> int { const int j = pair_partner(i); return (j > i ? j : i) + 1; };
        [[maybe_unused]] auto pair_target = [&](int u, int i) -> int {
            const unsigned gu = (unsigned)g0 + (unsigned)u, gc = (unsigned)g0 + (unsigned)i;
            if (pair_partner(u) < 0 || (gu & 1u)) return u;
            return (((gu >> 1) ^ gu ^ (gc >> 1) ^ gc) & 1u) ? u + 1 : u;
        };
        [[maybe_unused]] auto pair_next = [&](bool to_twin, int &f, int &fn) -> bool {
            if (to_twin) gi = pair_partner(gi);
            else {
                const int u = pair_unit_end(gi);
                if (u >= glen) return false;
                gi = pair_target(u, gi);
            }
            tw_pending = !to_twin && pair_partner(gi) >= 0;
            const uint64_t vmask = s_vmask[tid < 16 * T ? tid : 0] & (has_var ? ~0ULL : 0ULL);
            const uint64_t g = (uint64_t)g0 + (unsigned)gi;
            f = sign_of_var(vmask, g ^ (g >> 1));
            const int u2 = pair_unit_end(gi);
            fn = f;
            if (u2 < glen) { const uint64_t gn = (uint64_t)g0 + (unsigned)pair_target(u2, gi); fn = sign_of_var(vmask, gn ^ (gn >> 1)); }
            return true;
        };
        for (;;) {
            [[maybe_unused]] const unsigned nunconv0 = nunconv;
            bool isfree = false;
            int f = 0;
            [[maybe_unused]] int fn = 0;
            if constexpr (NODE) {
                const int code = has_var ? (int)p.node_code[((size_t)chain * clen + gi) * p.node_ld + tid] : 0;
                isfree = code == 2;
                f = isfree ? 0 : code;
            } else {
                const uint64_t vmask = s_vmask[tid < 16 * T ? tid : 0] & (has_var ? ~0ULL : 0ULL);
                const uint64_t g = (uint64_t)g0 + (unsigned)gi, gn = g + 1;
                f = sign_of_var(vmask, g ^ (g >> 1));
                if constexpr (MERGED) fn = glen > 1 ? sign_of_var(vmask, gn ^ (gn >> 1)) : f;
                if constexpr (PAIR) {
                    tw_pending = pair_partner(0) >= 0;
                    const int u2 = pair_unit_end(0);
                    fn = f;
                    if (u2 < glen) { const uint64_t g2 = (uint64_t)g0 + (unsigned)pair_target(u2, 0); fn = sign_of_var(vmask, g2 ^ (g2 >> 1)); }
                }
            }
            blocked = false;
            int ninf_best = n + 1, patience = 3, rounds = 0;
            bool progress = false;
            for (;;) {
                if (progress) blocked = false;
                progress = false;
                const int par = sc & 1;
                ++sc;
                bool bad = false;
                [[maybe_unused]] bool nxt = false;
                if (has_var) {
                    const double fq = q * (double)(f > 1 ? 1 : (f < -1 ? -1 : f));
                    if (NODE && isfree) bad = !basic && !blocked && (fabs(q) > p.tol);
                    else if (basic) bad = (f == 0) || (fq < -p.tol);
                    else bad = (fq > p.tol) && !blocked;
                    if constexpr (MERGED) {
                        const double fqn = q * (double)(fn > 1 ? 1 : (fn < -1 ? -1 : fn));
                        nxt = basic ? ((fn == 0) || (fqn < -p.tol)) : (fqn > p.tol);
                    }
                }
                const unsigned long long bb = __ballot(bad), bs = __ballot(basic);
                unsigned summ = (unsigned)__popcll(bb);
#pragma unroll
                for (int sub = 0; sub < 4; ++sub)
                    if ((bb >> (16 * sub)) & 0xFFFFull) summ |= 0x100u << sub;
                if constexpr (!MERGED) {
                    if (lane == 0 && wave < nwords) { s_inf[par * 8 + wave] = bb; s_bas[par * 8 + wave] = bs; s_sum[par * 8 + wave] = summ; }
                } else {
                    const unsigned long long bn = __ballot(nxt);
                    unsigned summ2 = (unsigned)__popcll(bn);
#pragma unroll
                    for (int sub = 0; sub < 4; ++sub)
                        if ((bn >> (16 * sub)) & 0xFFFFull) summ2 |= 0x100u << sub;
                    if (lane == 0 && wave < nwords) {
                        s_inf[par * 8 + wave] = bb; s_inf[16 + par * 8 + wave] = bn; s_bas[par * 8 + wave] = bs;
                        s_sum[par * 8 + wave] = ((unsigned long long)summ2 << 32) | summ;
                    }
                }
                STAMP(9);
                __syncthreads();
                STAMP(10);
                int count = 0;
                unsigned tiles = 0;
                [[maybe_unused]] int count2 = 0;
                [[maybe_unused]] unsigned tiles2 = 0;
#pragma unroll
                for (int w = 0; w < NW; ++w) {
                    const unsigned long long sw2 = s_sum[par * 8 + w];
                    const unsigned sw = (unsigned)__builtin_amdgcn_readfirstlane((int)sw2);
                    count += (int)(sw & 0xFFu);
                    tiles |= (sw >> 8) << (4 * w);
                    if constexpr (MERGED) {
                        const unsigned sn = (unsigned)__builtin_amdgcn_readfirstlane((int)(sw2 >> 32));
                        count2 += (int)(sn & 0xFFu);
                        tiles2 |= (sn >> 8) << (4 * w);
                    }
                }
                STAMP(0);
                int soff = par * 8;
                bool all = true;
                bool done = count == 0;
                if (!done) {
                    if (count < ninf_best) { ninf_best = count; patience = 3; }
                    else if (patience > 0) --patience;
                    else all = false;
                    if (++rounds > p.max_rounds) { ++nunconv; done = true; }
                }
                if (done) {
                    if constexpr (!MERGED) break;
                    finish_pattern(gi, count != 0);
                    if constexpr (PAIR) {
                        int tw = 0;
                        if (tw_pending) {
                            tw = 2;
                            if (count == 0) {
                                const int part = sc & 1;
                                ++sc;
                                const uint64_t vmask = s_vmask[tid < 16 * T ? tid : 0] & (has_var ? ~0ULL : 0ULL);
                                const uint64_t gt = (uint64_t)g0 + (unsigned)pair_partner(gi);
                                const int ft = sign_of_var(vmask, gt ^ (gt >> 1));
                                const double fqt = q * (double)(ft > 1 ? 1 : (ft < -1 ? -1 : ft));
                                const bool badt = has_var && (basic ? ((ft == 0) || (fqt < -p.tol)) : (fqt > p.tol));
                                const unsigned long long bt = __ballot(badt);
                                unsigned summt = (unsigned)__popcll(bt);
#pragma unroll
                                for (int sub = 0; sub < 4; ++sub)
                                    if ((bt >> (16 * sub)) & 0xFFFFull) summt |= 0x100u << sub;
                                if (lane == 0 && wave < nwords) { s_inf[part * 8 + wave] = bt; s_sum[part * 8 + wave] = summt; }
                                __syncthreads();
                                STAMP(15);
                                int countt = 0;
                                unsigned tilest = 0;
#pragma unroll
                                for (int w = 0; w < NW; ++w) {
                                    const unsigned sw = (unsigned)__builtin_amdgcn_readfirstlane((int)s_sum[part * 8 + w]);
                                    countt += (int)(sw & 0xFFu);
                                    tilest |= (sw >> 8) << (4 * w);
                                }
                                if (countt == 0) {
                                    record_twin(pair_partner(gi), corner, q, basic);
                                    tw = 0;
                                } else if (countt <= PAIR_MAXC) {
                                    tw = 3;
                                    pr_ncol = 0;
                                    all = true;
                                    tiles = tilest;
                                    soff = part * 8;
                                }
                            }
                        }
                        if (tw == 2) {
                            if (!pair_next(true, f, fn)) break;
                            blocked = false;
                            ninf_best = n + 1; patience = 3; rounds = 0;
                            continue;
                        }
                    }
                    if (!(PAIR && pr_ncol >= 0)) {
                    if constexpr (PAIR) { if (!pair_next(false, f, fn)) break; }
                    else if (++gi >= glen) break;
                    blocked = false;
                    ninf_best = n + 1; patience = 3; rounds = 0;
                    if constexpr (MERGED) {
                        if constexpr (!PAIR) {
                        const uint64_t vmask = s_vmask[tid < 16 * T ? tid : 0] & (has_var ? ~0ULL : 0ULL);
                        const uint64_t gn = (uint64_t)g0 + (unsigned)gi + 1;
                        f = fn;
                        fn = gi + 1 < glen ? sign_of_var(vmask, gn ^ (gn >> 1)) : f;
                        }
                        if (count2 == 0 || p.max_rounds < 1) continue;
                        ninf_best = count2; rounds = 1;
                        all = true;
                        tiles = tiles2;
                        soff += 16;
                    }
                    }
                }
                int single_k = -1;
                if (!all) {
#pragma unroll
                    for (int w = 0; w < NW; ++w) {
                        unsigned long long ww = s_inf[par * 8 + w];
                        ww = ((unsigned long long)(unsigned)__builtin_amdgcn_readfirstlane((int)(ww >> 32)) << 32) |
                             (unsigned)__builtin_amdgcn_readfirstlane((int)ww);
                        if (ww) single_k = (w << 6) + 63 - __builtin_clzll(ww);
                    }
                    tiles = 1u << (single_k >> 4);
                }
                tiles = (unsigned)__builtin_amdgcn_readfirstlane((int)tiles);
                [[maybe_unused]] unsigned tmask = 0;
                if constexpr (LANE_MASKS) {
                    const int tl = lane < T ? lane : 0, wl = tl >> 2, shl = 16 * (tl & 3);
                    tmask = (unsigned)((s_inf[soff + wl] >> shl) & 0xFFFFull) | ((unsigned)((s_bas[par * 8 + wl] >> shl) & 0xFFFFull) << 16);
                }

                [[maybe_unused]] bool chain_end = false;
                while (tiles) {
                    const int kappa = __builtin_ctz(tiles);
                    unsigned pmall, basm;
                    if constexpr (LANE_MASKS) {
                        const unsigned tm = (unsigned)__builtin_amdgcn_readlane((int)tmask, kappa);
                        pmall = tm & 0xFFFFu;
                        if (!all) pmall = 1u << (single_k & 15);
                        basm = tm >> 16;
                    } else {
                        const int wsel = kappa >> 2, sh = 16 * (kappa & 3);
                        pmall = (unsigned)((s_inf[soff + wsel] >> sh) & 0xFFFFull);
                        if (!all) pmall = 1u << (single_k & 15);
                        basm = (unsigned)__builtin_amdgcn_readfirstlane((int)((s_bas[par * 8 + wsel] >> sh) & 0xFFFFull));
                        pmall = (unsigned)__builtin_amdgcn_readfirstlane((int)pmall);
                    }
                    while (pmall) {
                        unsigned rest = 0;
                        if (__builtin_expect(__builtin_popcount(pmall) > MB && !(PAIR && pr_ncol >= 0), 0)) {
                            rest = pmall;
#pragma unroll
                            for (int i = 0; i < MB; ++i) rest &= rest - 1;
                        }
                        const unsigned pm = pmall & ~rest;
                        pmall = rest;
                        const int m = __builtin_popcount(pm);
                        const int bpar = bc & 1;
                        double *P = Pbase + bpar * MB * CW;
                        if constexpr (PAIR) {
                            if (pr_ncol >= 0) P = Pbase + pr_ncol * CW;
                            else ++bc;
                        } else ++bc;
                        int kap = kappa;
                        asm volatile("" : "+s"(kap));
                        STAMP(12);
#define PARTLS_G(i) if constexpr (i < T) { if (__builtin_expect(kap == i, 0)) gather_tile<T, H, W, i>(S, P, a, b, pm); }
                        PARTLS_CASES(PARTLS_G)
#undef PARTLS_G
                        STAMP(13);
                        if (tid < 16 * T && (tid >> 4) == kappa && ((pm >> (tid & 15)) & 1u))
                            P[__builtin_popcount(pm & ((1u << (tid & 15)) - 1u)) * CW + RHSPOS] = q;
                        if constexpr (PAIR) {
                            if (pr_ncol >= 0 && tid < 16 * T && (tid >> 4) == kappa && ((pm >> (tid & 15)) & 1u))
                                s_cpos[pr_ncol + __builtin_popcount(pm & ((1u << (tid & 15)) - 1u))] = basic ? ~mypos : mypos;
                        }
                        int myj = -1;
                        bool my_basic = false;
                        if (rowrho == kappa && rowc < 16 && ((pm >> rowc) & 1u)) {
                            myj = __builtin_popcount(pm & ((1u << rowc) - 1u));
                            my_basic = (basm >> rowc) & 1u;
                        }
                        STAMP(8);
                        __syncthreads();
                        STAMP(1);
                        if (tid == 0) s_veto[bpar ^ 1] = NO_VETO;
                        if (!(PAIR && pr_ncol >= 0)) {
                            int veto;
                            switch (m) {
#define PARTLS_PB(i) case i: if constexpr (i <= MB) veto = panel_block<(i <= MB ? i : 1), CW, MB>(P, Z, U, Dinv, myj, my_basic, p.piv_eps, tid, tid, idle_wave); else veto = 0; break;
                                PARTLS_PB(1) PARTLS_PB(2) PARTLS_PB(3) PARTLS_PB(4) PARTLS_PB(5) PARTLS_PB(6) PARTLS_PB(7) PARTLS_PB(8)
                                PARTLS_PB(9) PARTLS_PB(10) PARTLS_PB(11) PARTLS_PB(12) PARTLS_PB(13) PARTLS_PB(14) PARTLS_PB(15)
#undef PARTLS_PB
                                default: veto = panel_block<MB, CW, MB>(P, Z, U, Dinv, myj, my_basic, p.piv_eps, tid, tid, idle_wave); break;
                            }
                            if (veto < m && tid != RHSPOS) atomicMin(&s_veto[bpar], veto);
                        }
                        STAMP(11);
                        __syncthreads();
                        STAMP(2);
                        const int vs = __builtin_amdgcn_readfirstlane(s_veto[bpar]);
                        unsigned pmx = pm;
                        int mx = m;
                        if (__builtin_expect(vs < m, 0)) {
                            unsigned r = pm;
                            for (int i = 0; i < vs; ++i) r &= r - 1;
                            const unsigned vbit = r & (0u - r);
                            blocked = blocked || (tid == 16 * kappa + __builtin_ctz(vbit));
                            pmall |= pm & ~vbit;
                            pmx = 0;
                            mx = 0;
                            ++nveto;
                        }
                        if constexpr (PAIR) {
                            const bool pr = pr_ncol >= 0;
                            pmx = pr ? 0u : pmx;
                            mx = pr ? 0 : mx;
                            pr_ncol += pr ? m : 0;
                        }
                        bool blk_ok = false;
#pragma unroll PARTLS_UPD_UNROLL
                        for (int s = 0; s < mx; ++s) {
                            const double inv = Dinv[s];
                            blk_ok = blk_ok || (inv != 0.0);
                            const double *Zs = Z + s * CW;
                            double x[L::XN];
#pragma unroll
                            for (int rho = 0; rho < L::XN; ++rho) x[rho] = Zs[a * RS + rho];
#pragma unroll
                            for (int gam = L::GLO; gam < L::GHI; ++gam) {
                                const double yg = -Zs[b * RS + gam] * inv;
#pragma unroll
                                for (int rho = 0; rho <= gam; ++rho)
                                    S[L::idx(rho, gam)] = fma(x[rho], yg, S[L::idx(rho, gam)]);
                            }
                            const double zr = Zs[RHSPOS], zri = zr * inv;
                            if (tid < 16 * T) q = fma(-Zs[mypos], zri, q);
                            corner = fma(-zr, zri, corner);
                        }
                        STAMP(3);
#define PARTLS_F(i) if constexpr (i < T) { if (__builtin_expect(kap == i, 0)) scatter_tile<T, H, W, i>(S, P, a, b, pmx); }
                        PARTLS_CASES(PARTLS_F)
#undef PARTLS_F
                        if (tid < 16 * T && (tid >> 4) == kappa && ((pmx >> (tid & 15)) & 1u)) {
                            const int j = __builtin_popcount(pmx & ((1u << (tid & 15)) - 1u));
                            q = P[j * CW + RHSPOS];
                            if (Dinv[j] != 0.0) basic = !basic;
                            else blocked = true;
                        }
                        progress = progress || blk_ok;
                        npiv += (unsigned)mx;
                        STAMP(4);
                    }
                    tiles &= tiles - 1;
                if constexpr (PAIR) {
                    if (pr_ncol >= 0 && tiles == 0) {
                        const int m = pr_ncol;
                        pr_ncol = -1;
                        const int part = (sc - 1) & 1;
                        int tidp = tid;
                        asm volatile("" : "+v"(tidp));
                        const int lanep = tidp & 63, wavep = __builtin_amdgcn_readfirstlane(tidp >> 6);
                        __syncthreads();
                        if (H == 0 && wavep == 3) pair_solve<CW>(Pbase, s_cpos, m, lanep, RHSPOS, s_pair);
                        __syncthreads();
                        const bool guard = __builtin_amdgcn_readfirstlane(__double2hiint(s_pair[2 * PAIR_MAXC + 1])) != 0;
                        const unsigned long long cw = s_inf[part * 8 + wavep];
                        const bool in_c = has_var && ((cw >> lanep) & 1ull);
                        double qt = q, cornert = corner;
                        {
                            const int rp = tidp < 16 * T ? (tidp & 15) * RS + (tidp >> 4) : RHSPOS;
                            for (int j = 0; j < m; ++j) {
                                const double aj = s_pair[j];
                                qt = fma(-Pbase[j * CW + rp], aj, qt);
                                cornert = fma(-Pbase[j * CW + RHSPOS], aj, cornert);
                            }
                        }
                        if (in_c) {
                            int rank = __popcll(cw & ((1ull << lanep) - 1ull));
#pragma unroll
                            for (int w = 0; w < NW; ++w)
                                if (w < wavep) rank += __popcll(s_inf[part * 8 + w]);
                            qt = s_pair[PAIR_MAXC + rank];
                        }
                        const bool bt = basic != in_c;
                        const uint64_t vmask = s_vmask[tidp < 16 * T ? tidp : 0] & (has_var ? ~0ULL : 0ULL);
                        const uint64_t gt = (uint64_t)g0 + (unsigned)pair_partner(gi);
                        const int ft = sign_of_var(vmask, gt ^ (gt >> 1));
                        const double fqt = qt * (double)(ft > 1 ? 1 : (ft < -1 ? -1 : ft));
                        const bool bad2 = has_var && (bt ? ((ft == 0) || (fqt < -p.tol)) : (fqt > p.tol));
                        const unsigned long long b2 = __ballot(bad2);
                        if (lanep == 0) s_tw[wavep] = b2 != 0ull;
                        __syncthreads();
                        int left = guard ? 1 : 0;
#pragma unroll
                        for (int w = 0; w < 8; ++w) left |= s_tw[w];
                        left = __builtin_amdgcn_readfirstlane(left);
                        if (!left) record_twin(pair_partner(gi), cornert, qt, bt);
                        STAMP(14);
                        if (!pair_next(left != 0, f, fn)) chain_end = true;
                        else {
                            blocked = false;
                            ninf_best = n + 1; patience = 3; rounds = 0;
                            if (!left && count2 != 0 && p.max_rounds >= 1) {
                                ninf_best = count2; rounds = 1;
                                all = true;
                                tiles = (unsigned)__builtin_amdgcn_readfirstlane((int)tiles2);
                                soff = par * 8 + 16;
                                const int tl = lanep < T ? lanep : 0, wl = tl >> 2, shl = 16 * (tl & 3);
                                tmask = (unsigned)((s_inf[soff + wl] >> shl) & 0xFFFFull) | ((unsigned)((s_bas[par * 8 + wl] >> shl) & 0xFFFFull) << 16);
                            }
                        }
                    }
                }
                }
                if constexpr (PAIR) {
                    if (chain_end) break;
                }
            }
            if constexpr (!MERGED) {
                finish_pattern(gi, nunconv != nunconv0);
                if (++gi >= glen) break;
            } else break;
        }
        if constexpr (NODE) {
            if (has_var) p.node_sol[(size_t)chain * p.node_ld + tid] = basic ? q : 0.0;
            if (tid == 0) p.node_obj2[chain] = corner;
            if (p.node_dst) {
                double *snap = p.node_dst[chain];
                if (snap && (H == 0 || T > 1)) {
                    tiles_store<L>(snap, S, t8);
                    if (tid < 16 * T) {
                        snap[(size_t)nslots(T) * 256 + tid] = q;
                        reinterpret_cast<int8_t *>(snap + (nslots(T) * 256 + 16 * T + 8))[tid] = basic ? 1 : 0;
                    }
                    if (tid == 0) snap[(size_t)nslots(T) * 256 + 16 * T] = corner;
                }
            }
            if (p.node_tab && (H == 0 || T > 1)) {
                double *tab = p.node_tab + (size_t)chain * (nslots(T) * 256 + 16 * T + 8);
                tiles_store<L>(tab, S, t8);
                if (tid < 16 * T) p.node_basic[(size_t)chain * 16 * T + tid] = basic ? 1 : 0;
            }
        }
    }
    STAMP_FLUSH;
    __syncthreads();
    if (tid == 0) {
        p.best_obj[blockIdx.x] = sqrt(s_best[0]);
        p.best_pat[blockIdx.x] = reinterpret_cast<long long *>(s_best)[1];
        if (p.second_obj) { p.second_obj[blockIdx.x] = sqrt(s_best[2]); p.second_pat[blockIdx.x] = reinterpret_cast<long long *>(s_best)[3]; }
        if (p.n_pivots && npiv) atomicAdd(p.n_pivots, (unsigned long long)npiv);
        if (p.n_unconverged && nunconv) atomicAdd(p.n_unconverged, (unsigned long long)nunconv);
        if (p.n_vetoes && nveto) atomicAdd(p.n_vetoes, (unsigned long long)nveto);
    }
}

__device__ __forceinline__ void batch_select(SweepParams &p)
{
    const int64_t q = blockIdx.y;
    p.T0 += q * p.batch_t0;
    p.tol = p.batch_tol[q];
    const int64_t o = q * p.batch_out;
    p.best_obj += o;
    p.best_pat += o;
    if (p.second_obj) { p.second_obj += o; p.second_pat += o; }
    if (p.n_unconverged) p.n_unconverged += o;
    if (p.n_pivots) p.n_pivots += o;
    if (p.n_vetoes) p.n_vetoes += o;
    if (p.best_sol) p.best_sol += q * (int64_t)gridDim.x * p.node_ld;
}

template <int T, bool NODE, bool MODELS = false, bool BATCH = false, bool PAIRK = false>
__global__ __launch_bounds__(THREADS, 2) void sweep_blk_kernel(SweepParams p)
{
    if constexpr (BATCH) batch_select(p);
    const int half = __builtin_amdgcn_readfirstlane((int)(threadIdx.x >> 8));
    if (half == 0) sweep_body<T, 0, NODE, 2, MODELS, BATCH, PAIRK>(p);
    else sweep_body<T, 1, NODE, 2, MODELS, BATCH, PAIRK>(p);
}
constexpr bool pair_compiled(int T) { return PARTLS_PAIR && PARTLS_MERGED_SCAN && PARTLS_LANE_MASKS && T > MAXT_S && T <= 16; }

#ifndef PARTLS_SMALL_OCC
#define PARTLS_SMALL_OCC(T) ((T) <= 8 ? 3 : 2)
#endif
template <int T, bool NODE, bool MODELS = false, bool BATCH = false>
__global__ __launch_bounds__(256, PARTLS_SMALL_OCC(T)) void sweep_small_kernel(SweepParams p)
{
    if constexpr (BATCH) batch_select(p);
    sweep_body<T, 0, NODE, 1, MODELS, BATCH>(p);
}

__global__ void layout_reg_kernel(const double *__restrict__ Tfull, int n, int T, double *__restrict__ out, int64_t in_stride, int64_t out_stride)
{
    const int64_t q = blockIdx.y;
    const int ld = n + 1;
    const int ns = T * (T + 1) / 2;
    const int idx = blockIdx.x * blockDim.x + threadIdx.x;
    const int tot = ns * 256 + 16 * T + 1;
    if (idx >= tot) return;
    const double *Tq = Tfull + q * in_stride;
    double *oq = out + q * out_stride;
    if (idx < ns * 256) {
        const int s = idx >> 8, t8 = idx & 255, a = t8 & 15, b = t8 >> 4;
        int gam = 0;
        while ((gam + 1) * (gam + 2) / 2 <= s) ++gam;
        const int rho = s - gam * (gam + 1) / 2;
        const int i = 16 * rho + a, j = 16 * gam + b;
        oq[idx] = (i < n && j < n) ? Tq[(size_t)i * ld + j] : ((i == j) ? 1.0 : 0.0);
    } else if (idx < ns * 256 + 16 * T) {
        const int v = idx - ns * 256;
        oq[idx] = (v < n) ? Tq[(size_t)v * ld + n] : 0.0;
    } else {
        oq[idx] = Tq[(size_t)n * ld + n];
    }
}

}

bool sweep_reg_supported(int n) { return n >= 1 && n <= 16 * blk::MAXT; }
int sweep_reg_tiles(int n) { return (n + 15) / 16; }
bool sweep_reg_exports(int T) { return PARTLS_EXPORT_BIG != 0 && T <= blk::EXPORT_MAXT; }
bool sweep_reg_small(int T) { return T <= blk::MAXT_S; }
size_t sweep_reg_t0_doubles(int T) { return (size_t)T * (T + 1) / 2 * 256 + 16 * (size_t)T + 8; }

hipError_t launch_layout_reg_batch(const double *Tfull, int n, int T, int batch, double *T0reg, hipStream_t s)
{
    const int tot = T * (T + 1) / 2 * 256 + 16 * T + 1;
    hipLaunchKernelGGL(blk::layout_reg_kernel, dim3((tot + 255) / 256, batch), dim3(256), 0, s, Tfull, n, T, T0reg,
                       (int64_t)(n + 1) * (n + 1), (int64_t)sweep_reg_t0_doubles(T));
    return hipGetLastError();
}

hipError_t launch_layout_reg(const double *Tfull, int n, int T, double *T0reg, hipStream_t s)
{
    return launch_layout_reg_batch(Tfull, n, T, 1, T0reg, s);
}

template <class R, class F>
static R dispatch_T(int T, R none, F f)
{
    switch (T) {
#ifdef PARTLS_ONLY_T
        case PARTLS_ONLY_T: return f(std::integral_constant<int, PARTLS_ONLY_T>{});
#else
#define PARTLS_L(i) case i + 1: return f(std::integral_constant<int, i + 1>{});
        PARTLS_CASES(PARTLS_L)
#undef PARTLS_L
#endif
        default: return none;
    }
}

template <int T>
static hipError_t launch_blk_batch_T(const SweepParams &p, int grid, int batch, hipStream_t s)
{
    if constexpr (T <= blk::MAXT_S) hipLaunchKernelGGL((blk::sweep_small_kernel<T, false, false, true>), dim3(grid, batch), dim3(256), 0, s, p);
    else hipLaunchKernelGGL((blk::sweep_blk_kernel<T, false, false, true>), dim3(grid, batch), dim3(blk::THREADS), 0, s, p);
    return hipGetLastError();
}

hipError_t launch_sweep_blk_batch(const SweepParams &p, int T, int grid, int batch, hipStream_t s)
{
    if (p.node_code || batch < 1 || batch > 65535) return hipErrorInvalidValue;
    return dispatch_T(T, hipErrorInvalidValue, [&](auto t) { return launch_blk_batch_T<decltype(t)::value>(p, grid, batch, s); });
}

template <int T>
static hipError_t launch_blk_T(const SweepParams &p, int grid, hipStream_t s, bool models)
{
    if constexpr (T <= blk::MAXT_S) {
        if (p.node_code) hipLaunchKernelGGL((blk::sweep_small_kernel<T, true>), dim3(grid), dim3(256), 0, s, p);
        else if (models) hipLaunchKernelGGL((blk::sweep_small_kernel<T, false, true>), dim3(grid), dim3(256), 0, s, p);
        else hipLaunchKernelGGL((blk::sweep_small_kernel<T, false>), dim3(grid), dim3(256), 0, s, p);
    } else {
        if (p.node_code) hipLaunchKernelGGL((blk::sweep_blk_kernel<T, true>), dim3(grid), dim3(blk::THREADS), 0, s, p);
        else if (models) hipLaunchKernelGGL((blk::sweep_blk_kernel<T, false, true>), dim3(grid), dim3(blk::THREADS), 0, s, p);
        else if (blk::pair_compiled(T) && p.pair) hipLaunchKernelGGL((blk::sweep_blk_kernel<T, false, false, false, blk::pair_compiled(T)>), dim3(grid), dim3(blk::THREADS), 0, s, p);
        else hipLaunchKernelGGL((blk::sweep_blk_kernel<T, false>), dim3(grid), dim3(blk::THREADS), 0, s, p);
    }
    return hipGetLastError();
}

template <int T>
static int concurrency_T()
{
    if constexpr (T <= blk::MAXT_S) {
        int n = 0;
        if (hipOccupancyMaxActiveBlocksPerMultiprocessor(&n, reinterpret_cast<const void *>(&blk::sweep_small_kernel<T, false>), 256, 0) != hipSuccess || n < 1) n = 1;
        return n;
    }
    return 1;
}
int sweep_reg_concurrency_query(int T);
int sweep_reg_concurrency(int T)
{
    static std::atomic<int> cached[blk::MAXT + 2];
    if (T >= 0 && T <= blk::MAXT) { const int v = cached[T].load(std::memory_order_relaxed); if (v > 0) return v; }
    const int v = sweep_reg_concurrency_query(T);
    if (T >= 0 && T <= blk::MAXT) cached[T].store(v, std::memory_order_relaxed);
    return v;
}
int sweep_reg_concurrency_query(int T)
{
    return dispatch_T(T, 1, [](auto t) { return concurrency_T<decltype(t)::value>(); });
}

hipError_t launch_sweep_blk(const SweepParams &p, int T, int grid, hipStream_t s, bool models)
{
    return dispatch_T(T, hipErrorInvalidValue, [&](auto t) { return launch_blk_T<decltype(t)::value>(p, grid, s, models); });
}

}
```

partitionedls.jl_amd/csrc/sweep_setup.hip:

```cpp
#include "ctx.h"
#include "near_tie.h"
#include "sweep_rules.h"
#include <algorithm>
#include <cmath>
#include <cstring>
#include <numeric>

namespace partls {

SweepParams sweep_params(const partls_ctx *c, bool internal_order)
{
    SweepParams p{};
    const bool permuted = internal_order && !c->order_identity;
    p.n = c->n; p.kbits = c->kbits;
    p.mask = permuted ? c->maskInt.as<uint64_t>() : c->maskTabP;
    p.scratch = c->scratch.as<double>();
    p.tol = c->tol; p.piv_eps = SWEEP_PIV_EPS; p.max_rounds = sweep_max_rounds(c->n);
    for (int k = 0; k < 40; ++k) p.rbit.gbit[k] = (uint8_t)k;
    if (permuted) for (int k = 0; k < c->kbits; ++k) p.rbit.gbit[c->order.gbit[k]] = (uint8_t)k;
    return p;
}

partls_status ensure_sweep_scratch(partls_ctx *c, int grid)
{
    const size_t ld = (size_t)c->n + 1;
    PARTLS_HIP_CHECK(c->scratch.ensure((c->use_reg ? 64 : (size_t)grid * ld * ld) * sizeof(double)));
    return PARTLS_OK;
}

partls_status node_sweep_params(partls_ctx *c, size_t nodes, int64_t chain_len, int grid, SweepParams *p)
{
    const size_t wgs = (size_t)std::max(grid, 4096);
    PARTLS_HIP_CHECK(c->bestObj.ensure(sizeof(double) * wgs));
    PARTLS_HIP_CHECK(c->bestPat.ensure(sizeof(int64_t) * wgs));
    *p = sweep_params(c, false);
    p->g_begin = 0; p->g_end = (int64_t)nodes; p->chain_len = chain_len;
    p->best_obj = c->bestObj.as<double>(); p->best_pat = c->bestPat.as<int64_t>();
    return PARTLS_OK;
}

void bind_sweep_block(SweepParams &p, double *base, int grid, bool runner_up)
{
    const SweepBlock b = sweep_block(base, grid, runner_up);
    bind_counters(p, b.counters);
    p.best_obj = b.best_obj; p.best_pat = b.best_pat;
    p.second_obj = b.second_obj; p.second_pat = b.second_pat;
}

hipError_t launch_any_sweep(partls_ctx *c, SweepParams &p, int grid, bool models)
{
    if (c->use_reg) {
        p.T0 = c->T0reg.as<double>();
        return launch_sweep_blk(p, c->T, grid, c->stream, models);
    }
    p.T0 = c->Tfull.as<double>();
    return c->knobs.eager_generic ? launch_sweep_generic(p, grid, c->stream, models) : launch_sweep_lazy(p, grid, c->stream, models);
}

void opt_codes(const partls_ctx *c, uint64_t pattern, std::vector<int8_t> &codes)
{
    codes.resize((size_t)c->n);
    for (int i = 0; i < c->n; ++i) {
        const int f = sign_of_var(c->mask_tab[(size_t)i], pattern);
        codes[(size_t)i] = (int8_t)((f > 0) - (f < 0));
    }
}

partls_status solve_nodes(partls_ctx *c, const std::vector<int8_t> &codes, size_t cnt, std::vector<double> &sols,
                          std::vector<double> &obj2, unsigned long long *unconv, bool resume, bool want_tab)
{
    c->tab_valid = false;
    const int n = c->n, ld = n + 1;
    sols.assign(cnt * (size_t)n, 0.0);
    obj2.assign(cnt, 0.0);
    if (unconv) *unconv = 0;
    if (cnt == 0) return PARTLS_OK;
    if (codes.size() != cnt * (size_t)n) { set_error("solve_nodes: code array has the wrong size"); return PARTLS_ERR_BAD_ARG; }
    const int grid = (int)std::min<size_t>(cnt, c->use_reg ? 2048 : 512);
    PARTLS_HIP_CHECK(c->nodeCode.ensure(cnt * (size_t)n));
    const size_t out_words = 4 + cnt + cnt * (size_t)n;
    PARTLS_HIP_CHECK(c->nodeSol.ensure(out_words * sizeof(double)));
    const bool coop = !c->use_reg && cnt == 1 && !c->knobs.no_coop && !c->coop_fallback;
    c->coop_fallback = false;
    if (coop) {
        const size_t need = ((size_t)2 * ld * ld + (size_t)n / 8 + 2) * sizeof(double);
        if (c->scratch.bytes < need) c->coop_state_valid = false;
        PARTLS_HIP_CHECK(c->scratch.ensure(need));
    } else {
        c->coop_state_valid = false;
        const partls_status ss = ensure_sweep_scratch(c, grid);
        if (ss != PARTLS_OK) return ss;
    }
    PARTLS_HIP_CHECK(hipMemsetAsync(c->nodeSol.p, 0, 4 * sizeof(unsigned long long), c->stream));
    PARTLS_HIP_CHECK(hipMemcpyAsync(c->nodeCode.p, codes.data(), cnt * (size_t)n, hipMemcpyHostToDevice, c->stream));
    SweepParams p;
    const partls_status ps = node_sweep_params(c, cnt, 1, grid, &p);
    if (ps != PARTLS_OK) return ps;
    bind_counters(p, c->nodeSol.as<unsigned long long>());
    p.node_code = c->nodeCode.as<int8_t>();
    p.node_obj2 = c->nodeSol.as<double>() + 4; p.node_sol = c->nodeSol.as<double>() + 4 + cnt; p.node_ld = n;
    const bool dump_reg = want_tab && cnt == 1 && c->use_reg, dump_coop = want_tab && coop;
    const bool dump = dump_reg || dump_coop;
    const size_t tabd = dump_reg ? sweep_reg_t0_doubles(c->T) : (dump_coop ? (size_t)ld * ld : 0);
    if (dump) {
        if (dump_reg) {
            PARTLS_HIP_CHECK(c->nodeTab.ensure(tabd * sizeof(double)));
            PARTLS_HIP_CHECK(c->nodeBasic.ensure((size_t)16 * c->T));
        }
        if (c->hTabDoubles < tabd) {
            c->hTabDoubles = 0;
            PARTLS_HIP_CHECK(c->hTab.alloc(tabd));
            PARTLS_HIP_CHECK(c->hBasic.alloc(1024 + 16 ));
            c->hTabDoubles = tabd;
        }
        if (dump_reg) { p.node_tab = c->nodeTab.as<double>(); p.node_basic = c->nodeBasic.as<int8_t>(); }
    }
    if (coop) {
        p.T0 = c->Tfull.as<double>();
        p.resume = (resume && c->coop_state_valid) ? 1 : 0;
        PARTLS_HIP_CHECK(c->gridCtr.ensure(64));
        p.grid_ctr = c->gridCtr.as<unsigned>();
        p.coop_fault = c->knobs.coop_fault;
        c->coop_state_valid = false;
        const int rows_wg = c->knobs.coop_rows > 0 ? c->knobs.coop_rows : 6;
        int nwg = (ld + rows_wg - 1) / rows_wg;
        if (nwg > 128) nwg = 128;
        PARTLS_HIP_CHECK(launch_sweep_coop(p, nwg, c->stream));
    } else {
        PARTLS_HIP_CHECK(launch_any_sweep(c, p, grid));
    }
    unsigned long long counters[4] = {0, 0, 0, 0};
    std::vector<double> outw_big;
    double *outw_buf;
    if (out_words <= ((size_t)64 << 20) / sizeof(double)) { PARTLS_HIP_CHECK(c->nodeOut.resize(out_words)); outw_buf = c->nodeOut.data(); }
    else { outw_big.resize(out_words); outw_buf = outw_big.data(); }
    const double *outw = outw_buf;
    PARTLS_HIP_CHECK(hipMemcpyAsync(outw_buf, c->nodeSol.p, out_words * sizeof(double), hipMemcpyDeviceToHost, c->stream));
    if (dump_reg) {
        PARTLS_HIP_CHECK(hipMemcpyAsync(c->hTab, c->nodeTab.p, tabd * sizeof(double), hipMemcpyDeviceToHost, c->stream));
        PARTLS_HIP_CHECK(hipMemcpyAsync(c->hBasic, c->nodeBasic.p, (size_t)16 * c->T, hipMemcpyDeviceToHost, c->stream));
    }
    if (dump_coop) {
        const char *flagbuf = static_cast<const char *>(c->scratch.p) + (size_t)2 * ld * ld * sizeof(double);
        PARTLS_HIP_CHECK(hipMemcpyAsync(c->hBasic, flagbuf, (size_t)n + 1, hipMemcpyDeviceToHost, c->stream));
        PARTLS_HIP_CHECK(hipStreamSynchronize(c->stream));
        const size_t img = (size_t)(c->hBasic[n] & 1) * ld * ld;
        PARTLS_HIP_CHECK(hipMemcpyAsync(c->hTab, c->scratch.as<double>() + img, tabd * sizeof(double), hipMemcpyDeviceToHost, c->stream));
    }
    PARTLS_HIP_CHECK(hipStreamSynchronize(c->stream));
    std::memcpy(counters, outw, sizeof(counters));
    if (coop && (counters[0] >> 40)) {
        c->coop_fallback = true;
        return solve_nodes(c, codes, cnt, sols, obj2, unconv, false, want_tab);
    }
    if (coop) c->coop_state_valid = counters[0] == 0;
    std::copy(outw + 4, outw + 4 + cnt, obj2.begin());
    std::copy(outw + 4 + cnt, outw + out_words, sols.begin());
    if (unconv) *unconv = counters[0];
    c->last_pivots = counters[1]; c->last_vetoes = counters[2]; c->last_blocks = counters[3];
    c->tab_valid = dump && counters[0] == 0;
    c->tab_full = dump_coop;
    return PARTLS_OK;
}

static partls_status nodes_on_stream(partls_ctx *c, const double *T0reg, double tol, size_t cnt, const int8_t *code, double *obj2,
                                     double *sol, unsigned long long *counters, int max_rounds)
{
    c->tab_valid = false;
    c->coop_state_valid = false;
    if (cnt == 0) return PARTLS_OK;
    const int n = c->n;
    const int grid = (int)std::min<size_t>(cnt, c->use_reg ? 2048 : 512);
    SweepParams p;
    partls_status st = ensure_sweep_scratch(c, grid);
    if (st == PARTLS_OK) st = node_sweep_params(c, cnt, 1, grid, &p);
    if (st != PARTLS_OK) return st;
    p.max_rounds = max_rounds;
    bind_counters(p, counters);
    p.node_code = code; p.node_obj2 = obj2; p.node_sol = sol; p.node_ld = n;
    if (T0reg) {
        p.T0 = T0reg; p.tol = tol;
        PARTLS_HIP_CHECK(launch_sweep_blk(p, c->T, grid, c->stream));
    } else {
        PARTLS_HIP_CHECK(launch_any_sweep(c, p, grid));
    }
    return PARTLS_OK;
}

partls_status solve_nodes_device(partls_ctx *c, size_t cnt, const int8_t *code, double *obj2, double *sol,
                                 unsigned long long *counters, int max_rounds)
{
    return nodes_on_stream(c, nullptr, 0.0, cnt, code, obj2, sol, counters, max_rounds);
}

partls_status solve_nodes_device_at(partls_ctx *c, const double *T0reg, double tol, size_t cnt, const int8_t *code, double *obj2,
                                    double *sol, unsigned long long *counters, int max_rounds)
{
    if (!c->use_reg || !T0reg) { set_error("solve_nodes_device_at: needs a register-kernel context and a tableau"); return PARTLS_ERR_STATE; }
    return nodes_on_stream(c, T0reg, tol, cnt, code, obj2, sol, counters, max_rounds);
}

}

using namespace partls;

partls_status partls::calibrate_bit_order(partls_ctx *c)
{
    const int kb = c->kbits, n = c->n;
    c->order_ready = true;
    c->order_identity = true;
    c->flip_cost.clear();
    for (int k = 0; k < 40; ++k) c->order.gbit[k] = (uint8_t)k;
    if (kb < 2 || c->knobs.bit_order == 1) return PARTLS_OK;
    const int ncu = c->ncu;
    const int nseg = kb >= 8 ? 2 : 1;
    const int seg_len = (kb + nseg - 1) / nseg, L = seg_len + 1;
    if (c->knobs.bit_order != 2 && ((int64_t)1 << kb) < (int64_t)ncu * 32 * (8 + seg_len)) return PARTLS_OK;
    const int chains = std::max(ncu - ncu % nseg, 2 * nseg);
    const size_t steps = (size_t)chains * L;

    PARTLS_HIP_CHECK(c->nodeCode.ensure(steps * (size_t)n));
    PARTLS_HIP_CHECK(c->nodePiv.ensure((3 * steps + 8) * sizeof(unsigned)));
    PARTLS_HIP_CHECK(c->nodeSol.ensure((4 + (size_t)chains + (size_t)chains * n) * sizeof(double)));
    SweepParams p;
    partls_status st = ensure_sweep_scratch(c, chains);
    if (st == PARTLS_OK) st = node_sweep_params(c, steps, L, chains, &p);
    if (st != PARTLS_OK) return st;
    PARTLS_HIP_CHECK(hipMemsetAsync(c->nodePiv.p, 0, 8 * sizeof(unsigned), c->stream));
    t_begin(c, PARTLS_T_CALIB);
    PARTLS_HIP_CHECK(launch_walk_codes(c->maskTabP, n, kb, chains, L, seg_len, nseg, c->nodeCode.as<int8_t>(), c->stream));
    p.n_unconverged = c->nodePiv.as<unsigned long long>();
    p.node_code = c->nodeCode.as<int8_t>();
    p.node_obj2 = c->nodeSol.as<double>() + 4; p.node_sol = c->nodeSol.as<double>() + 4 + chains; p.node_ld = n;
    p.node_piv = c->nodePiv.as<unsigned>() + 8;
    PARTLS_HIP_CHECK(launch_any_sweep(c, p, chains));
    t_end(c, PARTLS_T_CALIB);
    std::vector<unsigned> piv(3 * steps + 8);
    PARTLS_HIP_CHECK(hipMemcpyAsync(piv.data(), c->nodePiv.p, (3 * steps + 8) * sizeof(unsigned), hipMemcpyDeviceToHost, c->stream));
    PARTLS_HIP_CHECK(hipStreamSynchronize(c->stream));
    t_collect(c);
    c->coop_state_valid = false;
    c->tab_valid = false;
    unsigned long long unconv = 0;
    std::memcpy(&unconv, piv.data(), sizeof(unconv));
    if (unconv) return PARTLS_OK;

    const double ns = c->use_reg ? 0.5 * c->T * (c->T + 1) : 0.0;
    const double per_pivot = 730.0 + 4.4 * ns;
    const double w_block = c->use_reg ? c->knobs.cal_wb * 4400.0 / per_pivot : 0.0, w_scan = c->use_reg ? c->knobs.cal_ws * 2100.0 / per_pivot : 0.0;
    std::vector<double> cost((size_t)kb, 0.0);
    std::vector<int> cnt((size_t)kb, 0);
    for (int ch = 0; ch < chains; ++ch)
        for (int i = 1; i < L; ++i) {
            const int k = walk_flipped_bit(ch, i, kb, seg_len, nseg);
            const unsigned *now = &piv[8 + 3 * ((size_t)ch * L + i)], *was = now - 3;
            const double scans = (double)(now[2] - was[2]);
            cost[(size_t)k] += (double)(now[0] - was[0]) + w_block * (double)(now[1] - was[1]) + w_scan * (scans > 1.0 ? scans - 1.0 : 0.0);
            ++cnt[(size_t)k];
        }
    for (int k = 0; k < kb; ++k) cost[(size_t)k] = cnt[(size_t)k] ? cost[(size_t)k] / cnt[(size_t)k] : 0.0;
    std::vector<int> by_cost((size_t)kb);
    std::iota(by_cost.begin(), by_cost.end(), 0);
    std::stable_sort(by_cost.begin(), by_cost.end(), [&](int a, int b) { return cost[(size_t)a] < cost[(size_t)b]; });
    c->flip_cost = cost;
    double pred_ref = 0.0, pred_sorted = 0.0, wgt = 0.5;
    for (int b = 0; b < kb; ++b, wgt *= 0.5) { pred_ref += wgt * cost[(size_t)b]; pred_sorted += wgt * cost[(size_t)by_cost[(size_t)b]]; }
    if (c->knobs.bit_order != 2 && !(pred_sorted < 0.98 * pred_ref)) return PARTLS_OK;
    bool ident = true;
    for (int b = 0; b < kb; ++b) { c->order.gbit[by_cost[(size_t)b]] = (uint8_t)b; ident = ident && by_cost[(size_t)b] == b; }
    if (ident) return PARTLS_OK;
    std::vector<uint64_t> mi((size_t)n);
    for (int i = 0; i < n; ++i) {
        uint64_t m = c->mask_tab[(size_t)i], q = 0;
        for (; m; m &= m - 1) q |= 1ULL << c->order.gbit[__builtin_ctzll(m)];
        mi[(size_t)i] = q;
    }
    PARTLS_HIP_CHECK(c->maskInt.ensure((size_t)n * sizeof(uint64_t)));
    PARTLS_HIP_CHECK(hipMemcpyAsync(c->maskInt.p, mi.data(), (size_t)n * sizeof(uint64_t), hipMemcpyHostToDevice, c->stream));
    PARTLS_HIP_CHECK(hipStreamSynchronize(c->stream));
    c->order_identity = false;
    return PARTLS_OK;
}

int64_t partls::reference_pattern(const partls_ctx *c, int64_t q)
{
    if (q < 0 || c->order_identity) return q;
    uint64_t r = 0;
    for (int k = 0; k < c->kbits; ++k) r |= (((uint64_t)q >> c->order.gbit[k]) & 1ULL) << k;
    return (int64_t)r;
}

bool partls::sweep_pairs(const partls_ctx *c, int64_t total)
{
    if (!c->use_reg || sweep_reg_small(c->T) || c->T > 16 || c->knobs.pair == 0) return false;
    if (c->knobs.pair == 1) return true;
    const int kb = c->kbits, seg_len = (kb + (kb >= 8 ? 2 : 1) - 1) / (kb >= 8 ? 2 : 1);
    if (kb < 2 || ((int64_t)1 << kb) < (int64_t)c->ncu * 32 * (8 + seg_len) || total < (int64_t)c->ncu * 32) return false;
    int live = 0;
    for (int k = 0; k < kb; ++k)
        if (c->order.gbit[k] == 0)
            for (int i = 0; i < c->n; ++i) live += ((c->mask_tab[(size_t)i] >> k) & 1ULL) != 0 && c->hScale[(size_t)i] != 0.0;
    return live >= 12 && live <= 16;
}

bool partls::sweep_plan(partls_ctx *c, int64_t total, int64_t *chain_len_out, int *grid_out, const char *who)
{
    int64_t chain_len;
    if (c->knobs.chain_len > 0) chain_len = c->knobs.chain_len;
    else if (c->use_reg) {
        const int ncu = c->ncu;
        const int64_t per_chain = total >= (int64_t)ncu * 2048 * 8 ? 2048 : 1024;
        const int conc = sweep_reg_concurrency(c->T);
        if (conc > 1) {
            const int64_t slots = (int64_t)ncu * conc;
            const int64_t k = std::max<int64_t>(1, (total + slots * per_chain - 1) / (slots * per_chain));
            chain_len = std::max<int64_t>(4, (total + k * slots - 1) / (k * slots));
        } else {
        int64_t k = (total + (int64_t)ncu * per_chain - 1) / ((int64_t)ncu * per_chain);
        if (k < 2) k = 2;
        chain_len = (total + k * ncu - 1) / (k * ncu);
        if (chain_len < 16) chain_len = 16;
        }
    } else {
        const int ncu = c->ncu;
        chain_len = 256;
        while (chain_len > 16 && (total + chain_len - 1) / chain_len < ncu) chain_len >>= 1;
    }
    if (chain_len < 1) chain_len = 1;
    if (c->knobs.chain_len <= 0 && sweep_pairs(c, total)) chain_len += chain_len & 1;
    const int64_t nchains = (total + chain_len - 1) / chain_len;
    if (nchains >= (1LL << 31) || chain_len >= (1LL << 31)) { set_error("%s: more than 2^31 chains in one call; split the Gray-index range", who); return false; }
    int grid = (int)std::min<int64_t>(nchains, c->knobs.grid > 0 ? c->knobs.grid : (c->use_reg ? 4096 : 1024));
    if (grid < 1) grid = 1;
    *chain_len_out = chain_len;
    *grid_out = grid;
    return true;
}

void partls::install_sweep_result(partls_ctx *c, const double *sweep_out, int grid, bool has_sol, double *bobj_out, int64_t *bpat_out)
{
    const SweepBlock b = sweep_block(const_cast<double *>(sweep_out), grid, true);
    c->last_pivots = b.counters[1];
    c->last_vetoes = b.counters[2];
    c->sweep_vetoes = b.counters[2];
    c->export_wg = -1;
    std::vector<int64_t> bp((size_t)grid);
    double bobj = INFINITY;
    int64_t bpat = -1;
    int best_wg = -1;
    for (int i = 0; i < grid; ++i) {
        bp[(size_t)i] = reference_pattern(c, b.best_pat[i]);
        if (bp[(size_t)i] < 0) continue;
        if (bpat < 0 || b.best_obj[i] < bobj || (b.best_obj[i] == bobj && bp[(size_t)i] < bpat)) { bobj = b.best_obj[i]; bpat = bp[(size_t)i]; best_wg = i; }
    }
    if (has_sol) c->export_wg = best_wg;
    c->near_pat.clear();
    c->cand.clear();
    c->near_for = bpat;
    if (bpat >= 0) {
        const double yy = h_reg(c, (int)c->M + 1, (int)c->M + 1);
        const double lim2 = bobj * bobj + c->knobs.near_tie_rel * (yy > 0.0 ? yy : 0.0);
        std::vector<std::pair<double, int64_t>> others;
        for (int i = 0; i < grid; ++i) {
            if (bp[(size_t)i] >= 0) others.emplace_back(b.best_obj[i], bp[(size_t)i]);
            if (b.second_pat[i] >= 0) others.emplace_back(b.second_obj[i], reference_pattern(c, b.second_pat[i]));
        }
        install_near_ties({bobj, bpat}, std::move(others), lim2, 3, c->cand, c->near_pat, c->near_for);
    }
    *bobj_out = bobj;
    *bpat_out = bpat;
}
```

Baseline: 22.55 million.

## Add graded chain-length plan to balance tail of register sweep

Replaces uniform chain lengths in the register-tiled sweep with a graded plan: full-length chains first, then successively halved lengths per CU, so the final wave has short chains and less load-imbalance tail. A new chain kernel maps each block to its level's offset and length, and the grid equals the number of chains instead of being capped and looped. It also adds an env-var spec for explicit plans and optional per-chain clock instrumentation. The cost is more, shorter chains near the end, with more per-chain setup and lost warm-start reuse.

Result: no change. 22.77 million (median of 6 runs) (+1.0%).

```diff
diff --git a/partitionedls.jl_amd/csrc/api.hip b/partitionedls.jl_amd/csrc/api.hip
--- a/partitionedls.jl_amd/csrc/api.hip
+++ b/partitionedls.jl_amd/csrc/api.hip
@@ -82,6 +82,15 @@
     if (const char *e = getenv("PARTLS_TOL_REL")) c->knobs.tol_rel = atof(e);
     if (const char *e = getenv("PARTLS_CHAIN_LEN")) c->knobs.chain_len = atoll(e);
     if (const char *e = getenv("PARTLS_GRID")) c->knobs.grid = atoll(e);
+    if (!parse_chain_plan_spec(getenv("PARTLS_CHAIN_PLAN"), &c->knobs.chain_plan)) {
+        set_error("partls_create: PARTLS_CHAIN_PLAN=\"%s\" is neither auto, uniform nor a list LENxCOUNT,LENxCOUNT,... of at most %d levels",
+                  getenv("PARTLS_CHAIN_PLAN"), CHAIN_PLAN_MAX_LEVELS);
+        partls_destroy(c);
+        return PARTLS_ERR_BAD_ARG;
+    }
+#ifdef PARTLS_CHAIN_CLOCK
+    if (const char *e = getenv("PARTLS_CHAIN_CLOCK_FILE")) c->knobs.chain_clock_file = e;
+#endif
     if (const char *e = getenv("PARTLS_GRAM_S")) c->knobs.gram_S = atoi(e);
     if (const char *e = getenv("PARTLS_GRAM_CR")) c->knobs.gram_cr = atoi(e);
     if (const char *e = getenv("PARTLS_COOP_ROWS")) c->knobs.coop_rows = atoi(e);
diff --git a/partitionedls.jl_amd/csrc/chain_plan.h b/partitionedls.jl_amd/csrc/chain_plan.h
--- /dev/null
+++ b/partitionedls.jl_amd/csrc/chain_plan.h
@@ -0,0 +1,162 @@
+#pragma once
+#include <stdint.h>
+#include <stdlib.h>
+#include <string.h>
+
+namespace partls {
+
+constexpr int CHAIN_PLAN_MAX_LEVELS = 8;
+constexpr int64_t CHAIN_PLAN_MAX_CHAINS = 4096;
+constexpr int64_t CHAIN_PLAN_LMAX = 2048;
+constexpr int64_t CHAIN_PLAN_FLOOR = 64;
+constexpr int64_t CHAIN_PLAN_MIN_LEN = 16;
+constexpr int64_t CHAIN_PLAN_MIN_PER_CU = 2048;
+#ifndef PARTLS_CHAIN_PLAN_AUTO_GRADED
+#define PARTLS_CHAIN_PLAN_AUTO_GRADED 1
+#endif
+
+struct ChainLevel { int64_t first_chain, first_off, len, count; };
+struct ChainPlan {
+    int nlev;
+    ChainLevel lev[CHAIN_PLAN_MAX_LEVELS];
+    int64_t chain_len;
+    int64_t nchains;
+};
+
+enum { CHAIN_PLAN_AUTO = 0, CHAIN_PLAN_UNIFORM = 1, CHAIN_PLAN_EXPLICIT = 2 };
+struct ChainPlanSpec { int mode; int n; int64_t len[CHAIN_PLAN_MAX_LEVELS], count[CHAIN_PLAN_MAX_LEVELS]; };
+
+inline bool parse_chain_plan_spec(const char *s, ChainPlanSpec *out)
+{
+    memset(out, 0, sizeof(*out));
+    if (!s || !*s || !strcmp(s, "auto")) { out->mode = CHAIN_PLAN_AUTO; return true; }
+    if (!strcmp(s, "uniform")) { out->mode = CHAIN_PLAN_UNIFORM; return true; }
+    out->mode = CHAIN_PLAN_EXPLICIT;
+    const char *q = s;
+    for (;;) {
+        if (out->n >= CHAIN_PLAN_MAX_LEVELS) return false;
+        int64_t v[2] = {0, 0};
+        for (int k = 0; k < 2; ++k) {
+            if (*q < '0' || *q > '9') return false;
+            while (*q >= '0' && *q <= '9') { v[k] = v[k] * 10 + (*q - '0'); if (v[k] >= ((int64_t)1 << 31)) return false; ++q; }
+            if (k == 0) { if (*q != 'x') return false; ++q; }
+        }
+        if (v[0] < 1 || v[1] < 1) return false;
+        out->len[out->n] = v[0]; out->count[out->n] = v[1]; ++out->n;
+        if (*q == 0) return true;
+        if (*q != ',') return false;
+        ++q;
+    }
+}
+
+inline int64_t uniform_chain_len(int64_t total, int ncu, bool use_reg, int conc, bool pair, long long knob_chain_len)
+{
+    int64_t chain_len;
+    if (knob_chain_len > 0) chain_len = knob_chain_len;
+    else if (use_reg) {
+        const int64_t per_chain = total >= (int64_t)ncu * 2048 * 8 ? 2048 : 1024;
+        if (conc > 1) {
+            const int64_t slots = (int64_t)ncu * conc;
+            int64_t k = (total + slots * per_chain - 1) / (slots * per_chain);
+            if (k < 1) k = 1;
+            chain_len = (total + k * slots - 1) / (k * slots);
+            if (chain_len < 4) chain_len = 4;
+        } else {
+            int64_t k = (total + (int64_t)ncu * per_chain - 1) / ((int64_t)ncu * per_chain);
+            if (k < 2) k = 2;
+            chain_len = (total + k * ncu - 1) / (k * ncu);
+            if (chain_len < 16) chain_len = 16;
+        }
+    } else {
+        chain_len = 256;
+        while (chain_len > 16 && (total + chain_len - 1) / chain_len < ncu) chain_len >>= 1;
+    }
+    if (chain_len < 1) chain_len = 1;
+    if (knob_chain_len <= 0 && pair) chain_len += chain_len & 1;
+    return chain_len;
+}
+
+inline bool chain_levels_from_pairs(int64_t total, int n, const int64_t *len, const int64_t *count, ChainPlan *out)
+{
+    out->nlev = 0;
+    out->nchains = 0;
+    if (total < 1 || total >= ((int64_t)1 << 31) || n < 1 || n > CHAIN_PLAN_MAX_LEVELS) return false;
+    int64_t off = 0;
+    for (int i = 0; i < n && off < total; ++i) {
+        if (len[i] < 1 || count[i] < 1) return false;
+        int64_t cnt = count[i];
+        const int64_t need = (total - off + len[i] - 1) / len[i];
+        if (cnt > need) cnt = need;
+        if (out->nchains + cnt > CHAIN_PLAN_MAX_CHAINS) return false;
+        ChainLevel &l = out->lev[out->nlev++];
+        l.first_chain = out->nchains; l.first_off = off; l.len = len[i]; l.count = cnt;
+        out->nchains += cnt;
+        off += cnt * len[i];
+    }
+    return off >= total;
+}
+
+inline bool graded_chain_plan(int64_t total, int ncu, bool pair, int64_t lmax, int64_t floor_len, ChainPlan *out)
+{
+    out->nlev = 0;
+    out->nchains = 0;
+    if (ncu < 1 || lmax < floor_len || floor_len < CHAIN_PLAN_MIN_LEN || total / ncu < 4 * floor_len || total / ncu < CHAIN_PLAN_MIN_PER_CU) return false;
+    if (total / lmax > 2 * CHAIN_PLAN_MAX_CHAINS) return false;
+    int64_t len[CHAIN_PLAN_MAX_LEVELS], count[CHAIN_PLAN_MAX_LEVELS];
+    int n = 0;
+    const auto emit = [&](int64_t l, int64_t c) {
+        if (n > 0 && len[n - 1] == l) { count[n - 1] += c; return true; }
+        if (n == CHAIN_PLAN_MAX_LEVELS) return false;
+        len[n] = l; count[n] = c; ++n;
+        return true;
+    };
+    const auto half = [&](int64_t rem) { int64_t l = (rem + 2 * (int64_t)ncu - 1) / (2 * (int64_t)ncu); if (pair) l += l & 1; return l; };
+    int64_t rem = total;
+    while (rem > 2 * lmax * ncu) { if (!emit(lmax, ncu)) return false; rem -= lmax * ncu; }
+    int64_t l = half(rem);
+    while (l > floor_len) {
+        if (!emit(l, ncu)) return false;
+        rem -= l * ncu;
+        l = half(rem);
+    }
+    if (rem > 0) {
+        if (l < CHAIN_PLAN_MIN_LEN) return false;
+        if (!emit(l, (rem + l - 1) / l)) return false;
+    }
+    return chain_levels_from_pairs(total, n, len, count, out);
+}
+
+struct ChainPlanIn {
+    int64_t total;
+    int ncu;
+    bool use_reg;
+    int conc;
+    bool pair;
+    bool chain_mode;
+    long long knob_chain_len, knob_grid;
+};
+
+inline int chain_plan(const ChainPlanIn &in, const ChainPlanSpec &spec, ChainPlan *out)
+{
+    memset(out, 0, sizeof(*out));
+    out->chain_len = uniform_chain_len(in.total, in.ncu, in.use_reg, in.conc, in.pair, in.knob_chain_len);
+    out->nchains = (in.total + out->chain_len - 1) / out->chain_len;
+    const bool levels_ok = in.chain_mode && in.use_reg && in.conc == 1 && in.knob_chain_len <= 0 && in.knob_grid <= 0 && in.total >= 1 &&
+                           in.total < ((int64_t)1 << 31);
+    if (!levels_ok) return 0;
+    ChainPlan lv;
+    memset(&lv, 0, sizeof(lv));
+    lv.chain_len = out->chain_len;
+    if (spec.mode == CHAIN_PLAN_EXPLICIT) {
+        if (!chain_levels_from_pairs(in.total, spec.n, spec.len, spec.count, &lv)) return 1;
+        *out = lv;
+    } else if (spec.mode == CHAIN_PLAN_UNIFORM) {
+        const int64_t one_len = out->chain_len, one_count = out->nchains;
+        if (chain_levels_from_pairs(in.total, 1, &one_len, &one_count, &lv)) *out = lv;
+    } else if (PARTLS_CHAIN_PLAN_AUTO_GRADED) {
+        if (graded_chain_plan(in.total, in.ncu, in.pair, CHAIN_PLAN_LMAX, CHAIN_PLAN_FLOOR, &lv)) *out = lv;
+    }
+    return 0;
+}
+
+}
diff --git a/partitionedls.jl_amd/csrc/common.h b/partitionedls.jl_amd/csrc/common.h
--- a/partitionedls.jl_amd/csrc/common.h
+++ b/partitionedls.jl_amd/csrc/common.h
@@ -61,6 +61,16 @@
     const double *batch_tol;
 };
 
+struct ChainLevels {
+    int nlev, nchains;
+    int c0[8];
+    int len[8];
+    int off[8];
+#ifdef PARTLS_CHAIN_CLOCK
+    unsigned long long *clock;
+#endif
+};
+
 __device__ __forceinline__ bool ref_index_less(unsigned long long a, unsigned long long b, const unsigned char *rbit)
 {
     unsigned long long d = a ^ b;
@@ -76,7 +86,7 @@
 
 hipError_t launch_sweep_generic(const SweepParams &p, int grid, hipStream_t s, bool models = false);
 hipError_t launch_sweep_lazy(const SweepParams &p, int grid, hipStream_t s, bool models = false);
-hipError_t launch_sweep_blk(const SweepParams &p, int T, int grid, hipStream_t s, bool models = false);
+hipError_t launch_sweep_blk(const SweepParams &p, int T, int grid, hipStream_t s, bool models = false, const ChainLevels *lv = nullptr);
 hipError_t launch_sweep_blk_batch(const SweepParams &p, int T, int grid, int batch, hipStream_t s);
 hipError_t launch_layout_reg_batch(const double *Tfull, int n, int T, int batch, double *T0reg, hipStream_t s);
 hipError_t launch_sweep_coop(const SweepParams &p, int nwg, hipStream_t s);
diff --git a/partitionedls.jl_amd/csrc/ctx.h b/partitionedls.jl_amd/csrc/ctx.h
--- a/partitionedls.jl_amd/csrc/ctx.h
+++ b/partitionedls.jl_amd/csrc/ctx.h
@@ -1,5 +1,6 @@
 #pragma once
 #include "common.h"
+#include "chain_plan.h"
 #include <functional>
 #include <vector>
 
@@ -93,6 +94,7 @@
     double tol_rel = 1e-11;
     long long chain_len = 0;
     long long grid = 0;
+    partls::ChainPlanSpec chain_plan{};
     int gram_S = 0, gram_cr = 0;
     int coop_rows = 0;
     bool no_coop = false;
@@ -111,6 +113,9 @@
     bool alt_trace = false;
     bool alt_always_check = false;
     bool print_stamps = false;
+#ifdef PARTLS_CHAIN_CLOCK
+    std::string chain_clock_file;
+#endif
     int alt_ms_max_rounds = 0;
     long long alt_ms_chunk = 0;
     double kkt_tol = 1e-12;
@@ -152,6 +157,9 @@
     partls::DevBuf slab, G, maskAugD , scale, Tfull, T0reg, scratch, bestObj, bestSol , bestPat, counters, allOpt,
         wdev, partial, yhatD, gD, nodeCode, nodeSol, nodeObj, predX, predY, gridCtr, nodeTab, nodeBasic, altA, altGA, altHg,
         nodePiv, maskInt, allOptRef, bnbIn, bnbOut, altGersh, amsState, amsWork;
+#ifdef PARTLS_CHAIN_CLOCK
+    partls::DevBuf chainClock;
+#endif
     partls::DevChunks bnbChunks;
     size_t bnbSlotBytes = 0, bnbMaxSlots = 0;
     int bnbChunkSlots = 512;
@@ -230,9 +238,10 @@
             runner_up ? reinterpret_cast<int64_t *>(b + 3 * g) : nullptr};
 }
 void bind_sweep_block(SweepParams &p, double *base, int grid, bool runner_up);
-hipError_t launch_any_sweep(partls_ctx *c, SweepParams &p, int grid, bool models = false);
+hipError_t launch_any_sweep(partls_ctx *c, SweepParams &p, int grid, bool models = false, const ChainLevels *lv = nullptr);
 partls_status calibrate_bit_order(partls_ctx *c);
-bool sweep_plan(partls_ctx *c, int64_t total, int64_t *chain_len_out, int *grid_out, const char *who);
+bool sweep_plan(partls_ctx *c, int64_t total, int64_t *chain_len_out, int *grid_out, const char *who, bool chain_mode = false, ChainPlan *plan_out = nullptr);
+ChainLevels chain_levels_of(const ChainPlan &plan);
 bool sweep_pairs(const partls_ctx *c, int64_t total);
 int64_t reference_pattern(const partls_ctx *c, int64_t q);
 void install_sweep_result(partls_ctx *c, const double *sweep_out, int grid, bool has_sol, double *bobj_out, int64_t *bpat_out);
diff --git a/partitionedls.jl_amd/csrc/opt.hip b/partitionedls.jl_amd/csrc/opt.hip
--- a/partitionedls.jl_amd/csrc/opt.hip
+++ b/partitionedls.jl_amd/csrc/opt.hip
@@ -97,7 +97,9 @@
     const int64_t total = g_end - g_begin;
     int64_t chain_len = 0;
     int grid = 0;
-    if (!sweep_plan(c, total, &chain_len, &grid, "partls_opt_sweep")) return PARTLS_ERR_UNSUPPORTED;
+    ChainPlan plan;
+    if (!sweep_plan(c, total, &chain_len, &grid, "partls_opt_sweep", true, &plan)) return c->knobs.chain_plan.mode == CHAIN_PLAN_EXPLICIT ? PARTLS_ERR_BAD_ARG : PARTLS_ERR_UNSUPPORTED;
+    ChainLevels lv = chain_levels_of(plan);
 
     const size_t sweep_words = sweep_block_words(grid, true);
     PARTLS_HIP_CHECK(c->bestObj.ensure(sizeof(double) * sweep_block_words(std::max(grid, 4096), true)));
@@ -122,8 +124,17 @@
         p.node_ld = n;
     }
 
+#ifdef PARTLS_CHAIN_CLOCK
+    const bool clocked = !c->knobs.chain_clock_file.empty() && c->use_reg && !sweep_reg_small(c->T) && grid == (int)plan.nchains;
+    if (clocked) {
+        if (!lv.nlev) { lv.nlev = 1; lv.nchains = grid; lv.c0[0] = 0; lv.off[0] = 0; lv.len[0] = (int)chain_len; }
+        PARTLS_HIP_CHECK(c->chainClock.ensure((size_t)grid * 4 * sizeof(unsigned long long)));
+        PARTLS_HIP_CHECK(hipMemsetAsync(c->chainClock.p, 0, (size_t)grid * 4 * sizeof(unsigned long long), c->stream));
+        lv.clock = c->chainClock.as<unsigned long long>();
+    }
+#endif
     t_begin(c, PARTLS_T_SWEEP);
-    PARTLS_HIP_CHECK(launch_any_sweep(c, p, grid));
+    PARTLS_HIP_CHECK(launch_any_sweep(c, p, grid, false, &lv));
     t_end(c, PARTLS_T_SWEEP);
 
     unsigned long long cnt[3] = {0, 0, 0};
@@ -142,6 +153,15 @@
     PARTLS_HIP_CHECK(hipStreamSynchronize(c->stream));
     t_collect(c);
     std::memcpy(cnt, sweep_out, sizeof(cnt));
+#ifdef PARTLS_CHAIN_CLOCK
+    if (clocked) {
+        std::vector<unsigned long long> rec(2 + 2 * (size_t)lv.nlev + 4 * (size_t)grid);
+        rec[0] = (unsigned long long)grid; rec[1] = (unsigned long long)lv.nlev;
+        for (int l = 0; l < lv.nlev; ++l) { rec[2 + 2 * l] = (unsigned long long)lv.c0[l]; rec[3 + 2 * l] = (unsigned long long)lv.len[l]; }
+        PARTLS_HIP_CHECK(hipMemcpy(rec.data() + 2 + 2 * lv.nlev, c->chainClock.p, (size_t)grid * 4 * sizeof(unsigned long long), hipMemcpyDeviceToHost));
+        if (FILE *f = fopen(c->knobs.chain_clock_file.c_str(), "wb")) { fwrite(rec.data(), sizeof(unsigned long long), rec.size(), f); fclose(f); }
+    }
+#endif
     if (c->knobs.print_stamps) {
         double st[32] = {0};
         if (hipMemcpy(st, c->scratch.p, sizeof(st), hipMemcpyDeviceToHost) == hipSuccess)
@@ -355,7 +375,9 @@
         const int64_t cnt = std::min<int64_t>(piece, g_end - p0);
         int64_t chain_len = 0;
         int grid = 0;
-        if (!sweep_plan(c, cnt, &chain_len, &grid, "partls_opt_models")) return PARTLS_ERR_UNSUPPORTED;
+        ChainPlan plan;
+        if (!sweep_plan(c, cnt, &chain_len, &grid, "partls_opt_models", true, &plan)) return c->knobs.chain_plan.mode == CHAIN_PLAN_EXPLICIT ? PARTLS_ERR_BAD_ARG : PARTLS_ERR_UNSUPPORTED;
+        const ChainLevels lv = chain_levels_of(plan);
         PARTLS_HIP_CHECK(c->mdlCtr.ensure(sizeof(double) * sweep_block_words(grid, false)));
         PARTLS_HIP_CHECK(hipMemsetAsync(c->mdlCtr.p, 0, 4 * sizeof(unsigned long long), c->stream));
         const partls_status ss = ensure_sweep_scratch(c, grid);
@@ -365,7 +387,7 @@
         p.g_begin = p0; p.g_end = p0 + cnt; p.chain_len = chain_len;
         bind_sweep_block(p, c->mdlCtr.as<double>(), grid, false);
         p.node_sol = rows; p.node_obj2 = obj; p.node_ld = n;
-        PARTLS_HIP_CHECK(launch_any_sweep(c, p, grid, true));
+        PARTLS_HIP_CHECK(launch_any_sweep(c, p, grid, true, &lv));
         PARTLS_HIP_CHECK(launch_models_cleanup(rows, obj, p0, cnt, (int)M, (int)K, c->kbits, c->order, c->order_identity, c->permP,
                                                c->scale.as<double>(), c->maskAugD.as<uint64_t>(), raw_alpha != nullptr, out, c->stream));
         double *st = c->mdlStage.data();
diff --git a/partitionedls.jl_amd/csrc/sweep_blk.hip b/partitionedls.jl_amd/csrc/sweep_blk.hip
--- a/partitionedls.jl_amd/csrc/sweep_blk.hip
+++ b/partitionedls.jl_amd/csrc/sweep_blk.hip
@@ -69,6 +69,16 @@
 #define STAMP_DECL
 #define STAMP(ph) do { } while (0)
 #define STAMP_FLUSH do { } while (0)
+#endif
+
+#ifdef PARTLS_CHAIN_CLOCK
+#define CHAIN_CLOCK_START unsigned long long cc_t0 = 0; do { if constexpr (GRADED) { if (lv->clock && tid == THREADS - 1) cc_t0 = __builtin_amdgcn_s_memrealtime(); } } while (0)
+#define CHAIN_CLOCK_END do { if constexpr (GRADED) { if (lv->clock && tid == THREADS - 1) { unsigned long long *cc_o = lv->clock + 4 * (size_t)chain; \
+        cc_o[0] = cc_t0; cc_o[1] = __builtin_amdgcn_s_memrealtime(); cc_o[2] = __builtin_amdgcn_s_getreg((31 << 11) | 20); \
+        cc_o[3] = __builtin_amdgcn_s_getreg((31 << 11) | 4); } } } while (0)
+#else
+#define CHAIN_CLOCK_START do { } while (0)
+#define CHAIN_CLOCK_END do { } while (0)
 #endif
 
 static constexpr int CWMAX = colw(MAXT);
@@ -267,7 +277,7 @@
 #define PARTLS_CASES(M) M(0) M(1) M(2) M(3) M(4) M(5) M(6) M(7) M(8) M(9) M(10) M(11) M(12) M(13) M(14) M(15) M(16) M(17) M(18) M(19)
 
 template <int T, int H, bool NODE, int W = 2, bool MODELS = false, bool BATCH = false, bool PAIRK = false>
-__device__ __forceinline__ void sweep_body(const SweepParams &p)
+__device__ __forceinline__ void sweep_body(const SweepParams &p, [[maybe_unused]] const ChainLevels *lv = nullptr)
 {
     using L = Half<T, H, W>;
     constexpr int RS = L::RS, CW = L::CW, RHSPOS = 16 * RS, NW = (T + 3) / 4;
@@ -321,13 +331,30 @@
     unsigned npiv = 0, nunconv = 0, nveto = 0;
     unsigned bc = 0, sc = 0;
 
+    constexpr bool GRADED = !NODE && !BATCH && W == 2;
     const int clen = (int)p.chain_len;
-    const int nchains = (int)((p.g_end - p.g_begin + clen - 1) / clen);
+    int nchains = (int)((p.g_end - p.g_begin + clen - 1) / clen);
+    int chain = blockIdx.x;
+    int64_t g0 = 0;
+    int glen = 0;
+    const auto uniform_chain = [&] { g0 = p.g_begin + (int64_t)chain * clen; glen = (int)((g0 + clen < p.g_end) ? clen : p.g_end - g0); };
+    if constexpr (GRADED) {
+        uniform_chain();
+        if (lv->nlev) {
+            nchains = lv->nchains;
+            int c0 = 0, off = 0, len = lv->len[0];
+#pragma unroll
+            for (int l = 1; l < 8; ++l)
+                if (chain >= lv->c0[l]) { c0 = lv->c0[l]; off = lv->off[l]; len = lv->len[l]; }
+            g0 = p.g_begin + off + (int64_t)(chain - c0) * len;
+            glen = (int)((g0 + len < p.g_end) ? len : p.g_end - g0);
+        }
+    }
 
     STAMP_DECL
-    for (int chain = blockIdx.x; chain < nchains; chain += gridDim.x) {
-        const int64_t g0 = p.g_begin + (int64_t)chain * clen;
-        const int glen = (int)((g0 + clen < p.g_end) ? clen : p.g_end - g0);
+    for (; chain < nchains; chain += gridDim.x, GRADED ? uniform_chain() : void()) {
+        if constexpr (!GRADED) uniform_chain();
+        CHAIN_CLOCK_START;
         STAMP(5);
         const double *src = p.T0;
         if constexpr (NODE) {
@@ -365,7 +392,7 @@
             }
             if (p.all_opt && tid == THREADS - 1) p.all_opt[pat] = sqrt(obj2);
             if constexpr (MODELS) {
-                const size_t row = (size_t)chain * (size_t)clen + (size_t)gi;
+                const size_t row = (size_t)(g0 - p.g_begin) + (size_t)gi;
                 if (has_var) p.node_sol[row * p.node_ld + tid] = capped ? __builtin_nan("") : (basic ? q : 0.0);
                 if (tid == THREADS - 1) p.node_obj2[row] = capped ? __builtin_nan("") : sqrt(obj2);
             }
@@ -806,6 +833,7 @@
                 if (++gi >= glen) break;
             } else break;
         }
+        CHAIN_CLOCK_END;
         if constexpr (NODE) {
             if (has_var) p.node_sol[(size_t)chain * p.node_ld + tid] = basic ? q : 0.0;
             if (tid == 0) p.node_obj2[chain] = corner;
@@ -857,10 +885,18 @@
 template <int T, bool NODE, bool MODELS = false, bool BATCH = false, bool PAIRK = false>
 __global__ __launch_bounds__(THREADS, 2) void sweep_blk_kernel(SweepParams p)
 {
+    static_assert(NODE || BATCH, "chain mode runs sweep_blk_chain_kernel");
     if constexpr (BATCH) batch_select(p);
     const int half = __builtin_amdgcn_readfirstlane((int)(threadIdx.x >> 8));
     if (half == 0) sweep_body<T, 0, NODE, 2, MODELS, BATCH, PAIRK>(p);
     else sweep_body<T, 1, NODE, 2, MODELS, BATCH, PAIRK>(p);
+}
+template <int T, bool MODELS = false, bool PAIRK = false>
+__global__ __launch_bounds__(THREADS, 2) void sweep_blk_chain_kernel(SweepParams p, ChainLevels lv)
+{
+    const int half = __builtin_amdgcn_readfirstlane((int)(threadIdx.x >> 8));
+    if (half == 0) sweep_body<T, 0, false, 2, MODELS, false, PAIRK>(p, &lv);
+    else sweep_body<T, 1, false, 2, MODELS, false, PAIRK>(p, &lv);
 }
 constexpr bool pair_compiled(int T) { return PARTLS_PAIR && PARTLS_MERGED_SCAN && PARTLS_LANE_MASKS && T > MAXT_S && T <= 16; }
 
@@ -950,7 +986,7 @@
 }
 
 template <int T>
-static hipError_t launch_blk_T(const SweepParams &p, int grid, hipStream_t s, bool models)
+static hipError_t launch_blk_T(const SweepParams &p, int grid, hipStream_t s, bool models, const ChainLevels &lv)
 {
     if constexpr (T <= blk::MAXT_S) {
         if (p.node_code) hipLaunchKernelGGL((blk::sweep_small_kernel<T, true>), dim3(grid), dim3(256), 0, s, p);
@@ -958,9 +994,9 @@
         else hipLaunchKernelGGL((blk::sweep_small_kernel<T, false>), dim3(grid), dim3(256), 0, s, p);
     } else {
         if (p.node_code) hipLaunchKernelGGL((blk::sweep_blk_kernel<T, true>), dim3(grid), dim3(blk::THREADS), 0, s, p);
-        else if (models) hipLaunchKernelGGL((blk::sweep_blk_kernel<T, false, true>), dim3(grid), dim3(blk::THREADS), 0, s, p);
-        else if (blk::pair_compiled(T) && p.pair) hipLaunchKernelGGL((blk::sweep_blk_kernel<T, false, false, false, blk::pair_compiled(T)>), dim3(grid), dim3(blk::THREADS), 0, s, p);
-        else hipLaunchKernelGGL((blk::sweep_blk_kernel<T, false>), dim3(grid), dim3(blk::THREADS), 0, s, p);
+        else if (models) hipLaunchKernelGGL((blk::sweep_blk_chain_kernel<T, true>), dim3(grid), dim3(blk::THREADS), 0, s, p, lv);
+        else if (blk::pair_compiled(T) && p.pair) hipLaunchKernelGGL((blk::sweep_blk_chain_kernel<T, false, blk::pair_compiled(T)>), dim3(grid), dim3(blk::THREADS), 0, s, p, lv);
+        else hipLaunchKernelGGL((blk::sweep_blk_chain_kernel<T, false>), dim3(grid), dim3(blk::THREADS), 0, s, p, lv);
     }
     return hipGetLastError();
 }
@@ -989,9 +1025,11 @@
     return dispatch_T(T, 1, [](auto t) { return concurrency_T<decltype(t)::value>(); });
 }
 
-hipError_t launch_sweep_blk(const SweepParams &p, int T, int grid, hipStream_t s, bool models)
-{
-    return dispatch_T(T, hipErrorInvalidValue, [&](auto t) { return launch_blk_T<decltype(t)::value>(p, grid, s, models); });
-}
-
-}
+hipError_t launch_sweep_blk(const SweepParams &p, int T, int grid, hipStream_t s, bool models, const ChainLevels *lv)
+{
+    if (lv && lv->nlev && (p.node_code || sweep_reg_small(T) || grid != lv->nchains || lv->nlev > 8)) return hipErrorInvalidValue;
+    const ChainLevels none{};
+    return dispatch_T(T, hipErrorInvalidValue, [&](auto t) { return launch_blk_T<decltype(t)::value>(p, grid, s, models, lv ? *lv : none); });
+}
+
+}
diff --git a/partitionedls.jl_amd/csrc/sweep_setup.hip b/partitionedls.jl_amd/csrc/sweep_setup.hip
--- a/partitionedls.jl_amd/csrc/sweep_setup.hip
+++ b/partitionedls.jl_amd/csrc/sweep_setup.hip
@@ -2,6 +2,7 @@
 #include "near_tie.h"
 #include "sweep_rules.h"
 #include <algorithm>
+#include <climits>
 #include <cmath>
 #include <cstring>
 #include <numeric>
@@ -47,12 +48,13 @@
     p.second_obj = b.second_obj; p.second_pat = b.second_pat;
 }
 
-hipError_t launch_any_sweep(partls_ctx *c, SweepParams &p, int grid, bool models)
+hipError_t launch_any_sweep(partls_ctx *c, SweepParams &p, int grid, bool models, const ChainLevels *lv)
 {
     if (c->use_reg) {
         p.T0 = c->T0reg.as<double>();
-        return launch_sweep_blk(p, c->T, grid, c->stream, models);
-    }
+        return launch_sweep_blk(p, c->T, grid, c->stream, models, lv);
+    }
+    if (lv && lv->nlev) return hipErrorInvalidValue;
     p.T0 = c->Tfull.as<double>();
     return c->knobs.eager_generic ? launch_sweep_generic(p, grid, c->stream, models) : launch_sweep_lazy(p, grid, c->stream, models);
 }
@@ -303,38 +305,43 @@
     return live >= 12 && live <= 16;
 }
 
-bool partls::sweep_plan(partls_ctx *c, int64_t total, int64_t *chain_len_out, int *grid_out, const char *who)
-{
-    int64_t chain_len;
-    if (c->knobs.chain_len > 0) chain_len = c->knobs.chain_len;
-    else if (c->use_reg) {
-        const int ncu = c->ncu;
-        const int64_t per_chain = total >= (int64_t)ncu * 2048 * 8 ? 2048 : 1024;
-        const int conc = sweep_reg_concurrency(c->T);
-        if (conc > 1) {
-            const int64_t slots = (int64_t)ncu * conc;
-            const int64_t k = std::max<int64_t>(1, (total + slots * per_chain - 1) / (slots * per_chain));
-            chain_len = std::max<int64_t>(4, (total + k * slots - 1) / (k * slots));
-        } else {
-        int64_t k = (total + (int64_t)ncu * per_chain - 1) / ((int64_t)ncu * per_chain);
-        if (k < 2) k = 2;
-        chain_len = (total + k * ncu - 1) / (k * ncu);
-        if (chain_len < 16) chain_len = 16;
-        }
-    } else {
-        const int ncu = c->ncu;
-        chain_len = 256;
-        while (chain_len > 16 && (total + chain_len - 1) / chain_len < ncu) chain_len >>= 1;
-    }
-    if (chain_len < 1) chain_len = 1;
-    if (c->knobs.chain_len <= 0 && sweep_pairs(c, total)) chain_len += chain_len & 1;
-    const int64_t nchains = (total + chain_len - 1) / chain_len;
+bool partls::sweep_plan(partls_ctx *c, int64_t total, int64_t *chain_len_out, int *grid_out, const char *who, bool chain_mode, ChainPlan *plan_out)
+{
+    ChainPlanIn in{};
+    in.total = total; in.ncu = c->ncu; in.use_reg = c->use_reg;
+    in.conc = (c->use_reg && c->knobs.chain_len <= 0) ? sweep_reg_concurrency(c->T) : 1;
+    in.pair = c->knobs.chain_len <= 0 && sweep_pairs(c, total);
+    in.chain_mode = chain_mode && plan_out != nullptr;
+    in.knob_chain_len = c->knobs.chain_len; in.knob_grid = c->knobs.grid;
+    ChainPlan plan;
+    if (chain_plan(in, c->knobs.chain_plan, &plan) != 0) {
+        set_error("%s: PARTLS_CHAIN_PLAN does not fit a range of %lld Gray indices (patterns left uncovered, or more than %lld chains)", who,
+                  (long long)total, (long long)CHAIN_PLAN_MAX_CHAINS);
+        return false;
+    }
+    const int64_t chain_len = plan.chain_len, nchains = plan.nchains;
     if (nchains >= (1LL << 31) || chain_len >= (1LL << 31)) { set_error("%s: more than 2^31 chains in one call; split the Gray-index range", who); return false; }
     int grid = (int)std::min<int64_t>(nchains, c->knobs.grid > 0 ? c->knobs.grid : (c->use_reg ? 4096 : 1024));
+    if (plan.nlev) grid = (int)nchains;
     if (grid < 1) grid = 1;
     *chain_len_out = chain_len;
     *grid_out = grid;
+    if (plan_out) *plan_out = plan;
     return true;
+}
+
+ChainLevels partls::chain_levels_of(const ChainPlan &plan)
+{
+    ChainLevels lv{};
+    lv.nlev = plan.nlev;
+    lv.nchains = plan.nlev ? (int)plan.nchains : 0;
+    for (int l = 0; l < 8; ++l) {
+        const bool on = l < plan.nlev;
+        lv.c0[l] = on ? (int)plan.lev[l].first_chain : INT_MAX;
+        lv.len[l] = on ? (int)plan.lev[l].len : 0;
+        lv.off[l] = on ? (int)plan.lev[l].first_off : 0;
+    }
+    return lv;
 }
 
 void partls::install_sweep_result(partls_ctx *c, const double *sweep_out, int grid, bool has_sol, double *bobj_out, int64_t *bpat_out)
```
